# sidward14/gan-lab

Measured on AMD Instinct MI355X. Metric: images/sec (G+D step), StyleGAN 1024^2 bs32/GPU, higher is better.
Workload: dtype f32; 1 GPU; StyleGAN res_samples=1024 FFHQ-shaped synthetic, bs=32/GPU fp32, nonsaturating + R1(lambda=10) + drift, stabilised phase, 1 D-iter + 1 G-iter; global_batch=32, per_gpu_batch=32, parallelism=single

## Files before the change

### gan_lab_amd/_lib.py

```python
import ctypes
import os
import subprocess

import torch

_HERE = os.path.dirname(os.path.abspath(__file__))
CSRC = os.path.join(_HERE, 'csrc')
SO_PATH = os.path.join(CSRC, os.path.basename(os.environ.get('GANLAB_HIP_LIB', '') or 'libganlab_hip.so'))

_c_int, _c_ll, _c_f, _c_p, _c_sz, _c_u64 = (ctypes.c_int, ctypes.c_longlong, ctypes.c_float, ctypes.c_void_p,
                                             ctypes.c_size_t, ctypes.c_uint64)

ACT_NONE, ACT_LRELU = 0, 1
PACK_FWD, PACK_DGRAD = 0, 1


class ConvGeom(ctypes.Structure):
    _fields_ = [('N', _c_int), ('Cin', _c_int), ('Hin', _c_int), ('Win', _c_int),
                ('Cout', _c_int), ('ks', _c_int), ('pad', _c_int), ('up', _c_int), ('pool', _c_int)]


_GP = ctypes.POINTER(ConvGeom)


class PackDesc(ctypes.Structure):
    _fields_ = [('src', _c_p), ('dst', _c_p), ('kind', _c_int), ('Cout', _c_int), ('Cin', _c_int), ('ks', _c_int),
                ('mode', _c_int), ('up', _c_int), ('scale', _c_f), ('reserved', _c_int), ('total', _c_ll),
                ('block0', _c_ll)]

class SnJob(ctypes.Structure):
    _fields_ = [('w', _c_p), ('w_sn', _c_p), ('g_sn', _c_p), ('gw', _c_p), ('u', _c_p), ('v', _c_p), ('sigma', _c_p),
                ('tpart', _c_p), ('s', _c_p), ('dpart', _c_p), ('R', _c_int), ('K', _c_int), ('blk_t0', _c_ll),
                ('blk_s0', _c_ll), ('blk_e0', _c_ll)]


SN_ROW_CHUNK, SN_COL_TILE, SN_ELEM_BLOCK = 16, 1024, 2048


class OrthoJob(ctypes.Structure):
    _fields_ = [('w', _c_p), ('gw', _c_p), ('s', _c_p), ('q', _c_p), ('part', _c_p), ('penalty', _c_p), ('R', _c_int),
                ('K', _c_int), ('form', _c_int), ('n_part', _c_int), ('blk_g0', _c_ll), ('blk_a0', _c_ll)]


class EwmaJob(ctypes.Structure):
    _fields_ = [('dst', _c_p), ('src', _c_p), ('count', _c_ll)]


ORTHO_TILE, ORTHO_QROWS, ORTHO_ROW, ORTHO_COL = 64, 4, 0, 1


class HierJob(ctypes.Structure):
    _fields_ = [('w', _c_p), ('gw', _c_p), ('gw_own', _c_p), ('C', _c_int), ('z_off', _c_int), ('z_len', _c_int),
                ('col', _c_int), ('scale', _c_f), ('one', _c_f), ('blk_f0', _c_ll), ('blk_w0', _c_ll)]


SIGNATURES = {
    'ganlab_abi_version': (_c_int, []),
    'ganlab_last_launch': (_c_int, [ctypes.c_char_p, _c_int, ctypes.POINTER(ctypes.c_uint)]),
    'ganlab_launch_count': (ctypes.c_ulonglong, []),
    'ganlab_launch_history': (_c_int, [_c_int, ctypes.c_char_p, _c_int, ctypes.POINTER(ctypes.c_uint)]),
    'ganlab_conv_geom_size': (_c_int, []),
    'ganlab_conv_out_hw': (_c_int, [_GP, ctypes.POINTER(_c_int), ctypes.POINTER(_c_int)]),
    'ganlab_conv_pack_f32': (_c_ll, [_c_p, _c_p, _c_int, _c_int, _c_int, _c_int, _c_f, _c_p]),
    'ganlab_conv_fwd_f32': (_c_int, [_c_p, _c_p, _c_p, _c_p, _GP, _c_f, _c_int, _c_f, _c_p]),
    'ganlab_conv_dgrad_f32': (_c_int, [_c_p, _c_p, _c_p, _GP, _c_p]),
    'ganlab_conv_splitk_plan': (_c_int, [_GP, _c_int]),
    'ganlab_conv_fwd_splitk_f32': (_c_int, [_c_p, _c_p, _c_p, _c_p, _GP, _c_f, _c_int, _c_f, _c_p, _c_sz, _c_p]),
    'ganlab_conv_dgrad_splitk_f32': (_c_int, [_c_p, _c_p, _c_p, _GP, _c_p, _c_sz, _c_p]),
    'ganlab_conv_dgrad_mask_supported': (_c_int, [_GP]),
    'ganlab_conv_dgrad_mask_f32': (_c_int, [_c_p, _c_p, _c_p, _c_p, _GP, _c_f, _c_p]),
    'ganlab_conv_act_bwd_fused_supported': (_c_int, [_GP]),
    'ganlab_conv_dgrad_act_f32': (_c_int, [_c_p, _c_p, _c_p, _c_p, _GP, _c_f, _c_p]),
    'ganlab_conv_fwd_mask_f32': (_c_int, [_c_p, _c_p, _c_p, _c_p, _GP, _c_f, _c_p]),
    'ganlab_conv_wgrad_act_f32': (_c_int, [_c_p, _c_p, _c_p, _c_p, _c_p, _GP, _c_f, _c_f, _c_f, _c_p, _c_sz, _c_p]),
    'ganlab_conv_wgrad_workspace': (_c_sz, [_GP]),
    'ganlab_conv_wgrad_f32': (_c_int, [_c_p, _c_p, _c_p, _GP, _c_f, _c_p, _c_sz, _c_p]),
    'ganlab_conv_s2_supported': (_c_int, [_GP]),
    'ganlab_conv_s2_pack_f32': (_c_ll, [_c_p, _c_p, _c_int, _c_int, _c_int, _c_int, _c_f, _c_p]),
    'ganlab_conv_s2_fwd_f32': (_c_int, [_c_p, _c_p, _c_p, _c_p, _GP, _c_f, _c_int, _c_f, _c_p]),
    'ganlab_conv_s2_dgrad_f32': (_c_int, [_c_p, _c_p, _c_p, _GP, _c_p]),
    'ganlab_conv_s2_wgrad_workspace': (_c_sz, [_GP]),
    'ganlab_conv_s2_wgrad_f32': (_c_int, [_c_p, _c_p, _c_p, _GP, _c_f, _c_p, _c_sz, _c_p]),
    'ganlab_conv_bf16_supported': (_c_int, [_GP]),
    'ganlab_conv_pack_bf16': (_c_ll, [_c_p, _c_p, _c_int, _c_int, _c_int, _c_f, _c_p]),
    'ganlab_conv_fwd_bf16': (_c_int, [_c_p, _c_p, _c_p, _c_p, _GP, _c_f, _c_int, _c_f, _c_p]),
    'ganlab_conv_dgrad_bf16': (_c_int, [_c_p, _c_p, _c_p, _GP, _c_p]),
    'ganlab_conv_bf16_splitk_plan': (_c_int, [_GP, _c_int]),
    'ganlab_conv_fwd_bf16_splitk': (_c_int, [_c_p, _c_p, _c_p, _c_p, _GP, _c_f, _c_int, _c_f, _c_p, _c_sz, _c_p]),
    'ganlab_conv_dgrad_bf16_splitk': (_c_int, [_c_p, _c_p, _c_p, _GP, _c_p, _c_sz, _c_p]),
    'ganlab_conv_wgrad_bf16_workspace': (_c_sz, [_GP]),
    'ganlab_conv_wgrad_bf16': (_c_int, [_c_p, _c_p, _c_p, _GP, _c_f, _c_p, _c_sz, _c_p]),
    'ganlab_conv_x3_supported': (_c_int, [_GP, _c_int]),
    'ganlab_conv_x3_pack': (_c_ll, [_c_p, _c_p, _c_int, _c_int, _c_int, _c_f, _c_p]),
    'ganlab_conv_fwd_x3': (_c_int, [_c_p, _c_p, _c_p, _c_p, _GP, _c_f, _c_int, _c_f, _c_p]),
    'ganlab_conv_dgrad_x3': (_c_int, [_c_p, _c_p, _c_p, _GP, _c_p]),
    'ganlab_conv_dgrad_mask_x3': (_c_int, [_c_p, _c_p, _c_p, _c_p, _GP, _c_f, _c_p]),
    'ganlab_conv_fwd_aff_x3': (_c_int, [_c_p, _c_p, _c_p, _c_p, _c_p, _c_p, _GP, _c_f, _c_int, _c_f, _c_p]),
    'ganlab_conv_fwd_aff_tail_x3_chunks': (_c_int, [_GP]),
    'ganlab_conv_s2_x3_supported': (_c_int, [_GP, _c_int]),
    'ganlab_conv_s2_x3_pack': (_c_ll, [_c_p, _c_p, _c_int, _c_int, _c_int, _c_f, _c_p]),
    'ganlab_conv_s2_fwd_x3': (_c_int, [_c_p, _c_p, _c_p, _c_p, _GP, _c_f, _c_int, _c_f, _c_p]),
    'ganlab_conv_s2_fwd_aff_x3': (_c_int, [_c_p, _c_p, _c_p, _c_p, _c_p, _c_p, _GP, _c_f, _c_int, _c_f, _c_p]),
    'ganlab_conv_s2_dgrad_x3': (_c_int, [_c_p, _c_p, _c_p, _GP, _c_p]),
    'ganlab_conv_s2_down_x3_supported': (_c_int, [_GP, _c_int]),
    'ganlab_conv_s2_down_x3_pack': (_c_ll, [_c_p, _c_p, _c_int, _c_int, _c_int, _c_f, _c_p]),
    'ganlab_conv_s2_down_fwd_x3': (_c_int, [_c_p, _c_p, _c_p, _c_p, _GP, _c_f, _c_int, _c_f, _c_p]),
    'ganlab_conv_s2_down_dgrad_x3': (_c_int, [_c_p, _c_p, _c_p, _GP, _c_p]),
    'ganlab_conv_wgrad_x3_supported': (_c_int, [_GP]),
    'ganlab_conv_wgrad_x3_workspace': (_c_sz, [_GP]),
    'ganlab_conv_wgrad_x3': (_c_int, [_c_p, _c_p, _c_p, _c_p, _c_p, _GP, _c_f, _c_p, _c_sz, _c_p]),
    'ganlab_conv_s2_wgrad_x3_supported': (_c_int, [_GP]),
    'ganlab_conv_s2_wgrad_x3_workspace': (_c_sz, [_GP]),
    'ganlab_conv_s2_wgrad_x3': (_c_int, [_c_p, _c_p, _c_p, _c_p, _c_p, _GP, _c_f, _c_p, _c_sz, _c_p]),
    'ganlab_conv_fwd_aff_tail_x3': (_c_int, [_c_p, _c_p, _c_p, _c_p, _c_p, _c_p, _c_p, _c_p, _c_p, _c_p, _GP, _c_f, _c_int, _c_f,
                                             _c_f, _c_p, _c_sz, _c_p]),
    'ganlab_mask_bits_supported': (_c_int, [_c_int, _c_int]),
    'ganlab_blur3x3_bits_f32': (_c_int, [_c_p, _c_p, _c_p, _c_ll, _c_int, _c_int, _c_p]),
    'ganlab_blur_act_bwd_bits_f32': (_c_int, [_c_p, _c_p, _c_p, _c_p, _c_int, _c_int, _c_int, _c_int, _c_f, _c_f,
                                              _c_p, _c_sz, _c_p]),
    'ganlab_act_bwd_blur_bits_f32': (_c_int, [_c_p, _c_p, _c_p, _c_p, _c_p, _c_p, _c_int, _c_int, _c_int, _c_int,
                                              _c_f, _c_f, _c_p, _c_sz, _c_p]),
    'ganlab_conv_fwd_blur_supported': (_c_int, [_GP, _c_p, _c_p]),
    'ganlab_conv_fwd_blur_bits_f32': (_c_int, [_c_p, _c_p, _c_p, _c_p, _c_p, _GP, _c_f, _c_f, _c_p]),
    'ganlab_conv_s2_blur_supported': (_c_int, [_GP]),
    'ganlab_conv_s2_blur_workspace': (_c_sz, [_GP]),
    'ganlab_conv_s2_fwd_blur_tail_f32': (_c_int, [_c_p, _c_p, _c_p, _c_p, _c_p, _c_p, _c_p, _c_p, _c_p, _c_p, _GP, _c_f, _c_int,
                                                  _c_f, _c_f, _c_p, _c_sz, _c_p]),
    'ganlab_conv_s2_dgrad_blur_act_bits_f32': (_c_int, [_c_p, _c_p, _c_p, _c_p, _c_p, _GP, _c_f, _c_f, _c_p, _c_sz, _c_p]),
    'ganlab_conv_dgrad_rgb_sums_supported': (_c_int, [_GP, _c_int]),
    'ganlab_conv_dgrad_rgb_sums_workspace': (_c_sz, [_GP]),
    'ganlab_conv_dgrad_rgb_sums_f32': (_c_int, [_c_p, _c_p, _c_p, _c_p, _c_p, _c_p, _GP, _c_int, _c_f, _c_f, _c_f, _c_int, _c_int,
                                                _c_p, _c_sz, _c_p]),
    'ganlab_conv_fwd_bits_f32': (_c_int, [_c_p, _c_p, _c_p, _c_p, _c_p, _GP, _c_f, _c_int, _c_f, _c_p]),
    'ganlab_conv_dgrad_act_bits_f32': (_c_int, [_c_p, _c_p, _c_p, _c_p, _GP, _c_f, _c_p]),
    'ganlab_conv_fwd_mask_bits_f32': (_c_int, [_c_p, _c_p, _c_p, _c_p, _GP, _c_f, _c_p]),
    'ganlab_conv_wgrad_act_bits_f32': (_c_int, [_c_p, _c_p, _c_p, _c_p, _c_p, _GP, _c_f, _c_f, _c_f, _c_p, _c_sz, _c_p]),
    'ganlab_pack_desc_size': (_c_int, []),
    'ganlab_pack_many': (_c_int, [_c_p, _c_int, _c_ll, _c_p]),
    'ganlab_in_affine_f32': (_c_int, [_c_p, _c_p, _c_p, _c_p, _c_p, _c_int, _c_int, _c_p]),
    'ganlab_conv_aff_supported': (_c_int, [_GP]),
    'ganlab_conv_fwd_aff_f32': (_c_int, [_c_p, _c_p, _c_p, _c_p, _c_p, _c_p, _GP, _c_f, _c_int, _c_f, _c_p]),
    'ganlab_conv_fwd_aff_tail_chunks': (_c_int, [_GP]),
    'ganlab_conv_fwd_aff_tail_f32': (_c_int, [_c_p, _c_p, _c_p, _c_p, _c_p, _c_p, _c_p, _c_p, _c_p, _c_p, _GP, _c_f, _c_int, _c_f,
                                              _c_f, _c_p, _c_sz, _c_p]),
    'ganlab_conv_wgrad_aff_f32': (_c_int, [_c_p, _c_p, _c_p, _c_p, _c_p, _GP, _c_f, _c_p, _c_sz, _c_p]),
    'ganlab_conv_s2_aff_supported': (_c_int, [_GP]),
    'ganlab_conv_s2_fwd_aff_f32': (_c_int, [_c_p, _c_p, _c_p, _c_p, _c_p, _c_p, _GP, _c_f, _c_int, _c_f, _c_p]),
    'ganlab_conv_s2_wgrad_aff_f32': (_c_int, [_c_p, _c_p, _c_p, _c_p, _c_p, _GP, _c_f, _c_p, _c_sz, _c_p]),
    'ganlab_mod_conv_supported': (_c_int, [_GP]),
    'ganlab_mod_conv_stat_chunks': (_c_int, [_GP]),
    'ganlab_mod_conv_fwd_f32': (_c_int, [_c_p, _c_p, _c_p, _c_p, _c_p, _c_p, _c_p, _c_p, _c_p, _c_p, _GP, _c_f, _c_int,
                                         _c_f, _c_f, _c_p, _c_sz, _c_p]),
    'ganlab_mod_torgb_prep_f32': (_c_int, [_c_p, _c_p, _c_p, _c_p, _c_p, _c_p, _c_int, _c_int, _c_int, _c_f, _c_f, _c_p]),
    'ganlab_mod_torgb_wgrad_f32': (_c_int, [_c_p, _c_p, _c_p, _c_p, _c_p, _c_int, _c_int, _c_int, _c_f, _c_f, _c_p]),
    'ganlab_mod_torgb_fwd_f32': (_c_int, [_c_p, _c_p, _c_p, _c_p, _c_int, _c_int, _c_int, _c_ll, _c_p]),
    'ganlab_mod_torgb_cross_workspace': (_c_sz, [_c_int]),
    'ganlab_mod_torgb_cross_f32': (_c_int, [_c_p, _c_p, _c_p, _c_int, _c_int, _c_int, _c_ll, _c_p, _c_sz, _c_p]),
    'ganlab_blur3x3_f32': (_c_int, [_c_p, _c_p, _c_ll, _c_int, _c_int, _c_p]),
    'ganlab_up2_f32': (_c_int, [_c_p, _c_p, _c_ll, _c_int, _c_int, _c_f, _c_p]),
    'ganlab_pool2_f32': (_c_int, [_c_p, _c_p, _c_ll, _c_int, _c_int, _c_f, _c_p]),
    'ganlab_resample2d_f32': (_c_int, [_c_p, _c_p, _c_p, _c_p, _c_p, _c_p, _c_ll, _c_int, _c_int, _c_int, _c_int, _c_int,
                                       _c_int, _c_p]),
    'ganlab_bias_act_f32': (_c_int, [_c_p, _c_p, _c_p, _c_p, _c_p, _c_int, _c_int, _c_ll, _c_f, _c_int, _c_f, _c_p]),
    'ganlab_act_bwd_f32': (_c_int, [_c_p, _c_p, _c_p, _c_ll, _c_f, _c_p]),
    'ganlab_act_bwd_bias_f32': (_c_int, [_c_p, _c_p, _c_p, _c_p, _c_int, _c_int, _c_ll, _c_f, _c_f, _c_p, _c_sz, _c_p]),
    'ganlab_channel_sum_f32': (_c_int, [_c_p, _c_p, _c_p, _c_int, _c_int, _c_ll, _c_f, _c_p, _c_sz, _c_p]),
    'ganlab_channel_sum_workspace': (_c_sz, [_c_int, _c_int, _c_ll]),
    'ganlab_instnorm_stats_f32': (_c_int, [_c_p, _c_p, _c_p, _c_ll, _c_ll, _c_f, _c_p]),
    'ganlab_row_stats_workspace': (_c_sz, [_c_ll, _c_ll]),
    'ganlab_row_stats_f32': (_c_int, [_c_p, _c_p, _c_p, _c_ll, _c_ll, _c_f, _c_p, _c_sz, _c_p]),
    'ganlab_instnorm_style_fwd_f32': (_c_int, [_c_p, _c_p, _c_p, _c_p, _c_p, _c_int, _c_int, _c_ll, _c_p]),
    'ganlab_instnorm_style_bwd_reduce_f32': (_c_int, [_c_p, _c_p, _c_p, _c_p, _c_p, _c_p, _c_ll, _c_ll, _c_p]),
    'ganlab_instnorm_style_bwd_apply_f32': (_c_int, [_c_p, _c_p, _c_p, _c_p, _c_p, _c_p, _c_p, _c_p, _c_int, _c_int,
                                                     _c_ll, _c_p]),
    'ganlab_pixelnorm_fwd_f32': (_c_int, [_c_p, _c_p, _c_int, _c_int, _c_ll, _c_f, _c_p]),
    'ganlab_pixelnorm_bwd_f32': (_c_int, [_c_p, _c_p, _c_p, _c_int, _c_int, _c_ll, _c_f, _c_p]),
    'ganlab_blur_fused_supported': (_c_int, [_c_int, _c_int]),
    'ganlab_blur_fused_workspace': (_c_sz, [_c_int, _c_int, _c_int, _c_int]),
    'ganlab_blur_bias_act_f32': (_c_int, [_c_p, _c_p, _c_p, _c_p, _c_p, _c_int, _c_int, _c_int, _c_int, _c_f,
                                          _c_int, _c_f, _c_p]),
    'ganlab_blur_act_bwd_f32': (_c_int, [_c_p, _c_p, _c_p, _c_p, _c_int, _c_int, _c_int, _c_int, _c_f, _c_f,
                                         _c_p, _c_sz, _c_p]),
    'ganlab_act_bwd_blur_f32': (_c_int, [_c_p, _c_p, _c_p, _c_p, _c_p, _c_p, _c_int, _c_int, _c_int, _c_int,
                                         _c_f, _c_f, _c_p, _c_sz, _c_p]),
    'ganlab_act_stats_workspace': (_c_sz, [_c_int, _c_int, _c_ll]),
    'ganlab_bias_act_stats_f32': (_c_int, [_c_p, _c_p, _c_p, _c_p, _c_p, _c_p, _c_p, _c_int, _c_int, _c_ll, _c_f, _c_int,
                                           _c_f, _c_f, _c_p, _c_sz, _c_p]),
    'ganlab_blur_bias_act_stats_f32': (_c_int, [_c_p, _c_p, _c_p, _c_p, _c_p, _c_p, _c_p, _c_int, _c_int, _c_int, _c_int,
                                                _c_f, _c_int, _c_f, _c_f, _c_p, _c_sz, _c_p]),
    'ganlab_instnorm_bwd_act_workspace': (_c_sz, [_c_int, _c_int, _c_ll]),
    'ganlab_instnorm_style_bwd_act_f32': (_c_int, [_c_p] * 11 + [_c_int, _c_int, _c_ll, _c_int, _c_f, _c_f, _c_p, _c_sz,
                                                                 _c_p]),
    'ganlab_instnorm_bwd_rgb_supported': (_c_int, [_c_int, _c_int, _c_int, _c_ll]),
    'ganlab_instnorm_bwd_reduce_rgb_workspace': (_c_sz, [_c_int, _c_int, _c_ll]),
    'ganlab_instnorm_style_bwd_reduce_rgb_f32': (_c_int, [_c_p, _c_p, _c_int] + [_c_p] * 5 + [_c_int, _c_int, _c_ll, _c_p,
                                                                                            _c_sz, _c_p]),
    'ganlab_instnorm_style_bwd_act_rgb_f32': (_c_int, [_c_p, _c_p, _c_int] + [_c_p] * 10 + [_c_int, _c_int, _c_ll, _c_int,
                                                                                         _c_f, _c_f, _c_p, _c_sz, _c_p]),
    'ganlab_instnorm_style_bwd_act_blur_f32': (_c_int, [_c_p] * 11 + [_c_int, _c_int, _c_int, _c_int, _c_int, _c_f, _c_f,
                                                                      _c_p, _c_sz, _c_p]),
    'ganlab_u8_box_decode_f32': (_c_int, [_c_p, _c_p, _c_int, _c_int, _c_int, _c_int, _c_int, _c_p, _c_p, _c_p, _c_p]),
    'ganlab_chan_affine_f32': (_c_int, [_c_p, _c_p, _c_p, _c_p, _c_int, _c_int, _c_ll, _c_p]),
    'ganlab_mul_f32': (_c_int, [_c_p, _c_p, _c_p, _c_ll, _c_p]),
    'ganlab_ln_affine_fwd_f32': (_c_int, [_c_p, _c_p, _c_p, _c_p, _c_p, _c_p, _c_int, _c_ll, _c_int, _c_f, _c_p]),
    'ganlab_colscale_f32': (_c_int, [_c_p, _c_p, _c_p, _c_int, _c_ll, _c_p]),
    'ganlab_coldot_f32': (_c_int, [_c_p, _c_p, _c_p, _c_p, _c_p, _c_p, _c_int, _c_ll, _c_p]),
    'ganlab_ln_rowsums_workspace': (_c_sz, [_c_int, _c_ll]),
    'ganlab_ln_rowsums_f32': (_c_int, [_c_p, _c_p, _c_p, _c_p, _c_p, _c_p, _c_p, _c_p, _c_int, _c_ll, _c_p, _c_sz, _c_p, _c_p,
                                       _c_f, _c_p]),
    'ganlab_ln_project_f32': (_c_int, [_c_p, _c_p, _c_p, _c_p, _c_p, _c_p, _c_p, _c_p, _c_int, _c_ll, _c_p]),
    'ganlab_ln_bwd_cols_f32': (_c_int, [_c_p, _c_p, _c_p, _c_p, _c_p, _c_p, _c_p, _c_p, _c_p, _c_int, _c_ll, _c_p]),
    'ganlab_ln_bwdbwd_apply_f32': (_c_int, [_c_p, _c_p, _c_p, _c_p, _c_p, _c_p, _c_p, _c_p, _c_int, _c_ll, _c_p]),
    'ganlab_bn_stats_f32': (_c_int, [_c_p, _c_p, _c_int, _c_int, _c_ll, _c_p, _c_sz, _c_p]),
    'ganlab_bn_finalize_f32': (_c_int, [_c_p, _c_p, _c_p, _c_p, _c_p, _c_p, _c_int, _c_f, _c_f, _c_f, _c_p]),
    'ganlab_bn_apply_f32': (_c_int, [_c_p, _c_p, _c_p, _c_p, _c_p, _c_int, _c_int, _c_ll, _c_int, _c_f, _c_p]),
    'ganlab_bn_bwd_sums_f32': (_c_int, [_c_p, _c_p, _c_p, _c_p, _c_p, _c_int, _c_int, _c_ll, _c_p, _c_sz, _c_p, _c_p, _c_f,
                                        _c_p]),
    'ganlab_bn_bwd_apply_f32': (_c_int, [_c_p, _c_p, _c_p, _c_p, _c_p, _c_p, _c_p, _c_int, _c_int, _c_ll, _c_p]),
    'ganlab_tanh_fwd_f32': (_c_int, [_c_p, _c_p, _c_ll, _c_p]),
    'ganlab_tanh_bwd_f32': (_c_int, [_c_p, _c_p, _c_p, _c_ll, _c_p]),
    'ganlab_mbstd_fwd_f32': (_c_int, [_c_p, _c_p, _c_int, _c_int, _c_ll, _c_f, _c_p]),
    'ganlab_mbstd_bwd_f32': (_c_int, [_c_p, _c_p, _c_p, _c_int, _c_int, _c_ll, _c_f, _c_p]),
    'ganlab_mbstd_bwdbwd_f32': (_c_int, [_c_p, _c_p, _c_p, _c_p, _c_p, _c_int, _c_int, _c_ll, _c_f, _c_p]),
    'ganlab_axpby_f32': (_c_int, [_c_p, _c_p, _c_p, _c_ll, _c_f, _c_f, _c_p]),
    'ganlab_scale_dev_f32': (_c_int, [_c_p, _c_p, _c_p, _c_ll, _c_f, _c_p]),
    'ganlab_lerp_rows_f32': (_c_int, [_c_p, _c_p, _c_p, _c_p, _c_ll, _c_ll, _c_p]),
    'ganlab_sum_f32': (_c_int, [_c_p, _c_p, _c_ll, _c_f, _c_int, _c_p, _c_sz, _c_p]),
    'ganlab_sum_workspace': (_c_sz, [_c_ll]),
    'ganlab_bce_logits_fwd_f32': (_c_int, [_c_p, _c_p, _c_int, _c_f, _c_p]),
    'ganlab_bce_logits_bwd_f32': (_c_int, [_c_p, _c_p, _c_p, _c_int, _c_f, _c_p]),
    'ganlab_hinge_fwd_f32': (_c_int, [_c_p, _c_p, _c_int, _c_f, _c_f, _c_p]),
    'ganlab_hinge_bwd_f32': (_c_int, [_c_p, _c_p, _c_p, _c_int, _c_f, _c_f, _c_p]),
    'ganlab_chnorm_penalty_fwd_f32': (_c_int, [_c_p, _c_p, _c_int, _c_int, _c_ll, _c_f, _c_f, _c_p, _c_sz, _c_p]),
    'ganlab_chnorm_penalty_bwd_f32': (_c_int, [_c_p, _c_p, _c_p, _c_int, _c_int, _c_ll, _c_f, _c_f, _c_p]),
    'ganlab_adam_f32': (_c_int, [_c_p, _c_p, _c_p, _c_p, _c_ll, _c_f, _c_f, _c_f, _c_f, _c_f, _c_f, _c_f, _c_p]),
    'ganlab_ewma_f32': (_c_int, [_c_p, _c_p, _c_ll, _c_f, _c_p]),
    'ganlab_randn_f32': (_c_int, [_c_p, _c_ll, _c_u64, _c_u64, _c_p]),
    'ganlab_randn_dev_f32': (_c_int, [_c_p, _c_ll, _c_u64, _c_p, _c_u64, _c_p]),
    'ganlab_diffaug_params_f32': (_c_int, [_c_p, _c_int, _c_int, _c_int, _c_u64, _c_u64, _c_p]),
    'ganlab_diffaug_params_dev_f32': (_c_int, [_c_p, _c_int, _c_int, _c_int, _c_u64, _c_p, _c_u64, _c_p]),
    'ganlab_diffaug_fwd_workspace': (_c_sz, [_c_int, _c_int, _c_int, _c_int]),
    'ganlab_diffaug_bwd_workspace': (_c_sz, [_c_int, _c_int, _c_int, _c_int]),
    'ganlab_diffaug_fwd_f32': (_c_int, [_c_p, _c_p, _c_p, _c_int, _c_int, _c_int, _c_int, _c_p, _c_sz, _c_p]),
    'ganlab_diffaug_bwd_f32': (_c_int, [_c_p, _c_p, _c_p, _c_int, _c_int, _c_int, _c_int, _c_p, _c_sz, _c_p]),
    'ganlab_ada_params_f32': (_c_int, [_c_p, _c_int, _c_int, _c_int, _c_p, _c_int, _c_u64, _c_u64, _c_p]),
    'ganlab_ada_params_dev_f32': (_c_int, [_c_p, _c_int, _c_int, _c_int, _c_p, _c_int, _c_u64, _c_p, _c_u64, _c_p]),
    'ganlab_ada_fwd_f32': (_c_int, [_c_p, _c_p, _c_p, _c_int, _c_int, _c_int, _c_p]),
    'ganlab_ada_bwd_f32': (_c_int, [_c_p, _c_p, _c_p, _c_int, _c_int, _c_int, _c_p]),
    'ganlab_ada_update_f32': (_c_int, [_c_p, _c_p, _c_int, _c_int, _c_f, _c_f, _c_p]),
    'ganlab_swd_down_f32': (_c_int, [_c_p, _c_p, _c_ll, _c_int, _c_int, _c_p]),
    'ganlab_swd_band_f32': (_c_int, [_c_p, _c_p, _c_p, _c_ll, _c_int, _c_int, _c_p]),
# ... 149 lines not shown
```

### gan_lab_amd/csrc/common.h

```cpp
#pragma once
#include <hip/hip_runtime.h>
#include <stdint.h>

#include "../../include/ganlab_hip.h"

typedef float f32x4 __attribute__((ext_vector_type(4)));

static thread_local int gl_launch_status = GANLAB_OK;
extern thread_local const void* gl_last_kernel_fn;
extern thread_local unsigned gl_last_grid;
#define GL_LAUNCH_RING 16
extern thread_local const void* gl_ring_fn[GL_LAUNCH_RING];
extern thread_local unsigned gl_ring_grid[GL_LAUNCH_RING];
extern thread_local unsigned long long gl_launch_count;
#define GL_LAUNCH(k, grid, ...)                                                  \
  do {                                                                           \
    (void)hipGetLastError();                                                     \
    const dim3 gl_grid_ = (grid);                                                \
    gl_last_kernel_fn = reinterpret_cast<const void*>(k);                        \
    gl_last_grid = gl_grid_.x * gl_grid_.y * gl_grid_.z;                         \
    gl_ring_fn[gl_launch_count % GL_LAUNCH_RING] = gl_last_kernel_fn;            \
    gl_ring_grid[gl_launch_count % GL_LAUNCH_RING] = gl_last_grid;               \
    ++gl_launch_count;                                                           \
    hipLaunchKernelGGL(k, gl_grid_, __VA_ARGS__);                                \
    if (hipGetLastError() != hipSuccess) gl_launch_status = GANLAB_ELAUNCH;      \
  } while (0)
static inline int gl_take_status() {
  const int s = gl_launch_status;
  gl_launch_status = GANLAB_OK;
  return s;
}
#define GL_CHECK_LAUNCH() gl_take_status()

#include <cstdlib>
#define GL_ENV_ONCE(name) ([]() -> const char* { static const char* const v = getenv(name); return v; }())

static inline hipStream_t gl_stream(void* s) { return reinterpret_cast<hipStream_t>(s); }

__device__ __forceinline__ int gl_xcd_remap(int b, int n) {
  const int q = n >> 3, r = n & 7, xcd = b & 7, i = b >> 3;
  const int base = (xcd < r) ? xcd * (q + 1) : r * (q + 1) + (xcd - r) * q;
  return base + i;
}

__device__ __forceinline__ float gl_wave_sum(float v) {
#pragma unroll
  for (int o = 32; o > 0; o >>= 1) v += __shfl_xor(v, o, 64);
  return v;
}

__device__ __forceinline__ float gl_block_sum_256(float v, float* red) {
  v = gl_wave_sum(v);
  __syncthreads();
  if ((threadIdx.x & 63) == 0) red[threadIdx.x >> 6] = v;
  __syncthreads();
  return red[0] + red[1] + red[2] + red[3];
}

__device__ __forceinline__ double gl_block_sum_256d(double v, double* red) {
#pragma unroll
  for (int o = 32; o > 0; o >>= 1) v += __shfl_xor(v, o, 64);
  __syncthreads();
  if ((threadIdx.x & 63) == 0) red[threadIdx.x >> 6] = v;
  __syncthreads();
  return (red[0] + red[1]) + (red[2] + red[3]);
}

#ifndef GL_ACC_DUMP
#define GL_ACC_DUMP 1
#endif
#ifndef GL_ACC_DUMP_TERMS_V
#define GL_ACC_DUMP_TERMS_V 144
#endif
constexpr int GL_ACC_DUMP_TERMS = GL_ACC_DUMP_TERMS_V;

__device__ __forceinline__ void philox4x32_10(uint32_t c[4], uint32_t k0, uint32_t k1) {
#pragma unroll
  for (int r = 0; r < 10; ++r) {
    const uint64_t p0 = (uint64_t)0xD2511F53u * c[0], p1 = (uint64_t)0xCD9E8D57u * c[2];
    const uint32_t n0 = (uint32_t)(p1 >> 32) ^ c[1] ^ k0, n1 = (uint32_t)p1;
    const uint32_t n2 = (uint32_t)(p0 >> 32) ^ c[3] ^ k1, n3 = (uint32_t)p0;
    c[0] = n0; c[1] = n1; c[2] = n2; c[3] = n3;
    k0 += 0x9E3779B9u;
    k1 += 0xBB67AE85u;
  }
}

__device__ __forceinline__ float gl_lrelu(float v, float slope) { return v > 0.f ? v : v * slope; }

__device__ __forceinline__ float4 gl_few_dot(const float4 (&xv)[4], const float* __restrict__ wp, int Cin, int Cout_p, int co,
                                             float start) {
  float4 a = float4{start, start, start, start};
#pragma unroll
  for (int ci = 0; ci < 4; ++ci) {
    const float w = ci < Cin ? wp[(long long)ci * Cout_p + co] : 0.f;
    a.x += w * xv[ci].x; a.y += w * xv[ci].y; a.z += w * xv[ci].z; a.w += w * xv[ci].w;
  }
  return a;
}

struct gl_bf16x3 { __bf16 h, m, l; };
__device__ __forceinline__ gl_bf16x3 gl_split3(float v) {
  const __bf16 h = (__bf16)v;
  const float r1 = v - (float)h;
  const __bf16 m = (__bf16)r1;
  return gl_bf16x3{h, m, (__bf16)(r1 - (float)m)};
}

__device__ __forceinline__ void gl_x3_pack_position(const float* __restrict__ w9, bool flip, float scale, __bf16* __restrict__ out,
                                                    int CI, int ci, int co) {
  const int steps = CI / 32 * 9;
  const int ct = co >> 6, col = co & 63, c = ci >> 5, half = (ci >> 4) & 1, g = (ci >> 3) & 1, j = ci & 7;
#pragma unroll
  for (int t = 0; t < 9; ++t) {
    const int s = t < 8 ? (half ? 5 : 0) + (t >> 1) : 4;
    const int hi = t < 8 ? (t & 1) : half;
    const int kg = hi * 2 + g;
    float v = w9[flip ? 8 - t : t] * scale;
    asm volatile("" : "+v"(v));
    const gl_bf16x3 p = gl_split3(v);
    __bf16* base = out + (((long long)ct * steps + c * 9 + s) * (3 * 4 * 64)) * 8;
    base[((0 * 4 + kg) * 64 + col) * 8 + j] = p.h;
    base[((1 * 4 + kg) * 64 + col) * 8 + j] = p.m;
    base[((2 * 4 + kg) * 64 + col) * 8 + j] = p.l;
  }
}

__device__ __forceinline__ void gl_x3_up_pack_position(const float* __restrict__ w9, int up, float scale, __bf16* __restrict__ out,
                                                       int CI, int CO, int ci, int co) {
  const int nsteps = CI / 8;
  const bool c32 = (CO & 63) != 0;
  const int ct = c32 ? co >> 5 : co >> 6, j = ci & 7;
#pragma unroll
  for (int py = 0; py < 2; ++py)
#pragma unroll
    for (int px = 0; px < 2; ++px)
#pragma unroll
      for (int ty = 0; ty < 2; ++ty)
#pragma unroll
        for (int tx = 0; tx < 2; ++tx) {
          float v = 0.f;
#pragma unroll
          for (int ky = 0; ky < 3; ++ky)
#pragma unroll
            for (int kx = 0; kx < 3; ++kx) {
              const int ry = up ? ky : 2 - ky, rx = up ? kx : 2 - kx;
              const bool iny = py == 0 ? (ty == 0 ? ry == 0 : ry >= 1) : (ty == 0 ? ry <= 1 : ry == 2);
              const bool inx = px == 0 ? (tx == 0 ? rx == 0 : rx >= 1) : (tx == 0 ? rx <= 1 : rx == 2);
              if (iny && inx) v += w9[ky * 3 + kx];
            }
          v = v * (up ? scale : 0.25f * scale);
          asm volatile("" : "+v"(v));
          const gl_bf16x3 p = gl_split3(v);
          __bf16* base = out + (((c32 ? (long long)ct : (long long)ct * 2 + py) * nsteps + (ci >> 3)) * (3 * 4 * 128)) * 8;
          const int col = c32 ? py * 32 + (co & 31) : co & 63;
          const int kgq = ty * 2 + tx;
          base[((0 * 4 + kgq) * 128 + px * 64 + col) * 8 + j] = p.h;
          base[((1 * 4 + kgq) * 128 + px * 64 + col) * 8 + j] = p.m;
          base[((2 * 4 + kgq) * 128 + px * 64 + col) * 8 + j] = p.l;
        }
}

__device__ __forceinline__ float gl_comb_s2(int up, int a, int k) {
  if (up) {
    const int lo = (a == 0) ? 2 : (a == 1 ? 1 : 0), hi = (a == 0) ? 2 : (a == 1 ? 2 : (a == 2 ? 1 : 0));
    return (k >= lo && k <= hi) ? 1.f : 0.f;
  }
  const int lo = (a <= 1) ? 0 : (a == 2 ? 1 : 2), hi = (a == 0) ? 0 : (a == 1 ? 1 : 2);
  return (k >= lo && k <= hi) ? 0.5f : 0.f;
}
__device__ __forceinline__ void gl_x3_down_pack_position(const float* __restrict__ w9, int up, float scale, __bf16* __restrict__ out,
                                                         int CI, int ci, int co) {
  const int nsteps = CI / 8 * 4;
  const int ct = co >> 7, col = co & 127, q = ci >> 3, j = ci & 7;
  float k9[9];
#pragma unroll
  for (int t = 0; t < 9; ++t) k9[t] = w9[t];
#pragma unroll
  for (int a = 0; a < 4; ++a)
#pragma unroll
    for (int b = 0; b < 4; ++b) {
      float v = 0.f;
#pragma unroll
      for (int ky = 0; ky < 3; ++ky)
#pragma unroll
        for (int kx = 0; kx < 3; ++kx) v += gl_comb_s2(up, a, ky) * gl_comb_s2(up, b, kx) * k9[ky * 3 + kx];
      v = v * scale;
      asm volatile("" : "+v"(v));
      const gl_bf16x3 p = gl_split3(v);
      __bf16* base = out + (((long long)ct * nsteps + q * 4 + a) * (3 * 4 * 128)) * 8;
      base[((0 * 4 + b) * 128 + col) * 8 + j] = p.h;
      base[((1 * 4 + b) * 128 + col) * 8 + j] = p.m;
      base[((2 * 4 + b) * 128 + col) * 8 + j] = p.l;
    }
}

extern "C" int gl_tail_stats_finish(const double* spart, float* mean, float* rstd, long long planes, int chunks, double inv_hw, float eps,
                         hipStream_t st);

bool gl_wgrad_roll_supported(int N, int Cin, int Cout, int H, int W, int ks, int pad, int up, const void* x,
                             const void* gy);
int gl_wgrad_roll_slots(int N, int Cin, int Cout, int H, int W);
int gl_wgrad_roll_launch(const float* x, const float* gy, float* part, int N, int Cin, int Cout, int H, int W,
                         hipStream_t st, const float* aff_s = nullptr, const float* aff_t = nullptr);
bool gl_wgrad_s2_roll_supported(int N, int Cl, int Ch, int Hl, int Wl, const void* low, const void* high);
int gl_wgrad_s2_roll_slots(int N, int Cl, int Ch, int Hl, int Wl);
int gl_wgrad_s2_roll_launch(const float* low, const float* high, float* part, int N, int Cl, int Ch, int Hl, int Wl,
                            hipStream_t st, const float* aff_s = nullptr, const float* aff_t = nullptr);

bool gl_s2_roll_supported(int is_T, int N, int Cin, int Cout, int Hl, int Wl, const void* x, const void* y);
int gl_s2_roll_launch(int is_T, const float* x, const float* wp, const float* bias, float* y, int N, int Cin, int Cout,
                      int Hl, int Wl, int Cin_p, int Cout_p, float bias_scale, int act, float slope, hipStream_t st,
                      const float* aff_s = nullptr, const float* aff_t = nullptr);

bool gl_roll_blur_supported(int N, int Cin, int Cout, int H, int W, const void* x, const void* y);
int gl_roll_blur_launch(const float* x, const float* wp, const float* bias, float* y, void* bits, int N, int Cin, int Cout,
                        int H, int W, int Cin_p, int Cout_p, float bias_scale, float slope, hipStream_t st, int blur, int act);
```

### gan_lab_amd/csrc/conv_x3.hip

```cpp
#include "x3_common.h"

#include <type_traits>

#ifndef X3_EXP
#define X3_EXP 0
#endif

namespace {

constexpr int X3_NT = 64;
constexpr int X3_PL = 336;
constexpr int X3_HALF = 6 * X3_PL;
constexpr int X3_WSTEP = 3 * 4 * X3_NT;
constexpr int X3_AOFF = 0, X3_WOFF = 3 * X3_HALF;
constexpr int X3_WSTAGE = 2 * X3_WSTEP;
constexpr int X3_LDS = 3 * X3_HALF + 2 * X3_WSTAGE;

__host__ __device__ constexpr int x3_tap_lo(int s) { return s < 4 ? 2 * s : s == 4 ? 8 : 2 * (s - 5); }
__host__ __device__ constexpr int x3_tap_hi(int s) { return s < 4 ? 2 * s + 1 : s == 4 ? 8 : 2 * (s - 5) + 1; }
__host__ __device__ constexpr int x3_half_lo(int s) { return s <= 4 ? 0 : 1; }
__host__ __device__ constexpr int x3_half_hi(int s) { return s < 4 ? 0 : 1; }

__global__ void x3_pack_kernel(const float* __restrict__ w, __bf16* __restrict__ out, int Cout, int Cin, int mode, float scale) {
  const bool dg = mode == GANLAB_PACK_DGRAD;
  const int CO = dg ? Cin : Cout, CI = dg ? Cout : Cin;
  const long long e = blockIdx.x * (long long)blockDim.x + threadIdx.x;
  if (e >= (long long)CO * CI) return;
  const int col = (int)(e & 63);
  const long long t = e >> 6;
  const int ci = (int)(t % CI), ct = (int)(t / CI);
  const int co = ct * 64 + col;
  const float* w9 = dg ? w + ((long long)ci * Cin + co) * 9 : w + ((long long)co * Cin + ci) * 9;
  gl_x3_pack_position(w9, dg, scale, out, CI, ci, co);
}

struct X3Args {
  const float* x;
  const u32x4* wp;
  const float* bias;
  float* y;
  int N, CI, CO, H, W;
  int tiles_x, tiles_y, tiles_co, ntiles;
  float bias_scale, slope;
  int act;
  const float* mask;
  float mslope;
  const float* aff_s;
  const float* aff_t;
  const float* noise;
  const float* noise_w;
  double* spart;
};

constexpr int X3_PLAIN = 0, X3_MASK = 1, X3_AFF = 2, X3_AFF_TAIL = 3;

#define X3_ACC8(a) "+v"(a[0][0]), "+v"(a[0][1]), "+v"(a[1][0]), "+v"(a[1][1]), "+v"(a[2][0]), "+v"(a[2][1]), "+v"(a[3][0]), "+v"(a[3][1])

__host__ __device__ constexpr int x3_toff(int tap) { return (tap / 3) * 18 + tap % 3; }

struct X3Tile { int n, oy0, ox0, co_t; };

template <int FORM>
__global__ __launch_bounds__(512) void conv_x3_fwd_kernel(X3Args p) {
  constexpr bool MASK = FORM == X3_MASK, AFF = FORM == X3_AFF || FORM == X3_AFF_TAIL, TAIL = FORM == X3_AFF_TAIL;
  constexpr int NLOADS = AFF ? 6 : 4;
  __shared__ __attribute__((aligned(16))) u32x4 lds[X3_LDS];

  const int tid = threadIdx.x, lane = tid & 63;
  const int wv = __builtin_amdgcn_readfirstlane(tid >> 6);
  const int wm = wv >> 1, wn = wv & 1;
  const int l16 = lane & 15, kg = lane >> 4, lane16 = lane * 16;
  const int plane = p.H * p.W;
  const int nstages = p.CI / 64 * 9, ndc = p.CI / 64;
  const int G = gridDim.x;

  auto decode = [&](int t) {
    X3Tile c;
    c.co_t = t % p.tiles_co; t /= p.tiles_co;
    c.ox0 = (t % p.tiles_x) * 16; t /= p.tiles_x;
    c.oy0 = (t % p.tiles_y) * 16;
    c.n = t / p.tiles_y;
    return c;
  };

  const bool a_item = tid < 432;
  int a_pack;
  {
    const int e = a_item ? tid : 0;
    const int cq = e & 1;
    int t = e >> 1;
    const int cg = t % 6; t /= 6;
    const int r = t % 18, g = t / 18;
    const int unit48 = ((g * 3) * X3_PL + r * 18 + 4 * cg) * 16 + cq * 8;
    a_pack = unit48 | ((cg == 0 ? 3 : 0) << 16) | ((cg == 5 ? 1 : 4) << 18) | (r << 21) | (cg << 26) | ((g * 2 + cq) << 29);
  }
  const int cstride = plane * 4;
  f32x4 ar[4];
  f32x4 a_sv, a_tv;
  auto a_load = [&](const X3Tile& c, int half) {
    const u32x4 rs = x3_rsrc(p.x + (long long)c.n * p.CI * plane, (unsigned)((long long)p.CI * plane * 4));
    int pk = a_pack;
    asm volatile("" : "+v"(pk));
    const int ry = ((pk >> 21) & 31) - 1, rx = ((pk >> 26) & 7) * 4 - 4, a_ch = ((pk >> 29) & 3) * 4;
    const bool ok = a_item && (unsigned)(c.oy0 + ry) < (unsigned)p.H && (unsigned)(c.ox0 + rx) < (unsigned)p.W;
    const int off = ok ? (a_ch * plane + (c.oy0 + ry) * p.W + c.ox0 + rx) * 4 : (int)0x80000000;
    const int soff = half * 16 * plane * 4;
    if (X3_EXP & 4) return;
#pragma unroll
    for (int j = 0; j < 4; ++j) x3_ld(ar[j], rs, off + j * cstride, soff);
    if constexpr (AFF) {
      const unsigned tab = (unsigned)((long long)p.N * p.CI * 4);
      const u32x4 rss = x3_rsrc(p.aff_s, tab), rst = x3_rsrc(p.aff_t, tab);
      const int o = ok ? a_ch * 4 : (int)0x80000000;
      const int so = (c.n * p.CI + half * 16) * 4;
      x3_ld(a_sv, rss, o, so);
      x3_ld(a_tv, rst, o, so);
    }
  };
  auto a_wait = [&](auto younger) {
    if constexpr (AFF) x3_ld_wait<decltype(younger)::value>(ar, a_sv, a_tv); else x3_ld_wait<decltype(younger)::value>(ar);
  };
  auto a_store_px = [&](int slot, int i) {
    if (!a_item || (X3_EXP & 1)) return;
    int pk = a_pack;
    asm volatile("" : "+v"(pk));
    const int a_i0 = (pk >> 16) & 3, a_i1 = (pk >> 18) & 7;
    unsigned char* dst = reinterpret_cast<unsigned char*>(lds + X3_AOFF + slot * X3_HALF) + ((pk & 0x7fff) - 48);
    if (i < a_i0 || i >= a_i1) return;
    bf16x4 h, m, l;
#pragma unroll
    for (int j = 0; j < 4; ++j) {
      float v = i == 0 ? ar[j].x : i == 1 ? ar[j].y : i == 2 ? ar[j].z : ar[j].w;
      if constexpr (AFF) v = fmaf(v, j == 0 ? a_sv.x : j == 1 ? a_sv.y : j == 2 ? a_sv.z : a_sv.w,
                                  j == 0 ? a_tv.x : j == 1 ? a_tv.y : j == 2 ? a_tv.z : a_tv.w);
      x3_split_lane(v, j, h, m, l);
    }
    *reinterpret_cast<u32x2*>(dst + i * 16) = __builtin_bit_cast(u32x2, h);
    *reinterpret_cast<u32x2*>(dst + i * 16 + X3_PL * 16) = __builtin_bit_cast(u32x2, m);
    *reinterpret_cast<u32x2*>(dst + i * 16 + 2 * X3_PL * 16) = __builtin_bit_cast(u32x2, l);
  };
  auto a_store = [&](int slot) {
#pragma unroll
    for (int i = 0; i < 4; ++i) {
      a_store_px(slot, i);
      __builtin_amdgcn_sched_barrier(0);
    }
  };

  const __amdgpu_buffer_rsrc_t rs_w = __builtin_amdgcn_make_buffer_rsrc(
      const_cast<u32x4*>(p.wp), 0, (unsigned)((long long)p.tiles_co * nstages * X3_WSTAGE * 16), 0x00020000);
  auto w_dma = [&](const X3Tile& c, int st, int buf) {
    const int soff = (c.co_t * nstages + st) * (X3_WSTAGE * 16) + wv * 3072;
#pragma unroll
    for (int i = 0; i < 3; ++i)
      __builtin_amdgcn_raw_ptr_buffer_load_lds(rs_w, (__attribute__((address_space(3))) void*)(lds + X3_WOFF + buf * X3_WSTAGE + wv * 192 + i * 64),
                                               16, lane16, soff + i * 1024, 0, 0);
  };

  f32x4 accS[4][2], accH[4][2], accT[4][2];
#pragma unroll
  for (int m = 0; m < 4; ++m)
#pragma unroll
    for (int nn = 0; nn < 2; ++nn) {
      accS[m][nn] = f32x4{0.f, 0.f, 0.f, 0.f}; accH[m][nn] = f32x4{0.f, 0.f, 0.f, 0.f}; accT[m][nn] = f32x4{0.f, 0.f, 0.f, 0.f};
    }

  const int laneA = X3_AOFF + (kg & 1) * 3 * X3_PL + (4 * wm) * 18 + l16;
  const int laneB = X3_WOFF + kg * X3_NT + wn * 32 + l16;
  const bool khi = kg >= 2;
  const int khi_i = khi ? 1 : 0;

  bf16x8 aF[2][3], bF[2][2][3];
  auto a_frags = [&](int off, int m) {
#pragma unroll
    for (int pl = 0; pl < 3; ++pl) aF[m & 1][pl] = __builtin_bit_cast(bf16x8, lds[off + pl * X3_PL + m * 18]);
  };
  auto b_frags = [&](int buf, int step1, int nn, int set) {
#pragma unroll
    for (int pl = 0; pl < 3; ++pl)
      bF[set][nn][pl] = __builtin_bit_cast(bf16x8, lds[laneB + buf * X3_WSTAGE + step1 * X3_WSTEP + pl * 4 * X3_NT + nn * 16]);
  };

  int tile = gl_xcd_remap(blockIdx.x, G);
  if (tile >= p.ntiles) return;
  X3Tile cur = decode(tile);

  w_dma(cur, 0, 0);
  a_load(cur, 0); a_wait(std::integral_constant<int, 0>{}); a_store(0);
  a_load(cur, 1); a_wait(std::integral_constant<int, 0>{}); a_store(1);
  x3_barrier<0>();
  if (nstages > 1) w_dma(cur, 1, 1);
  int offA;
  {
    offA = laneA + (khi ? x3_toff(x3_tap_hi(0)) : x3_toff(x3_tap_lo(0)));
    a_frags(offA, 0);
    b_frags(0, 0, 0, 0);
    b_frags(0, 0, 1, 0);
  }

  int st = 0;
  int gst = 0;
  int r0 = 0;
  for (;;) {
    const int ntile = tile + G;
    const bool nvalid = ntile < p.ntiles;
    const X3Tile nxt = decode(nvalid ? ntile : tile);
    for (int dc = 0; dc < ndc; ++dc) {
      const int sl0 = r0, sl1 = r0 == 2 ? 0 : r0 + 1, sl2 = sl1 == 2 ? 0 : sl1 + 1;
      const bool lastdc = dc + 1 == ndc;
      const bool more = !lastdc || nvalid;
#pragma unroll
// ... 264 lines not shown
```

### gan_lab_amd/csrc/pack.hip

```cpp
#include "common.h"

namespace {

constexpr int round_up_c(int v, int m) { return (v + m - 1) / m * m; }

__global__ __launch_bounds__(256) void pack_many_kernel(const ganlab_pack_desc* __restrict__ descs, int n_desc) {
  int lo = 0, hi = n_desc - 1;
  const long long b = blockIdx.x;
  while (lo < hi) {
    const int mid = (lo + hi + 1) >> 1;
    if (descs[mid].block0 <= b) lo = mid; else hi = mid - 1;
  }
  const ganlab_pack_desc d = descs[lo];
  const long long e = (b - d.block0) * 256 + threadIdx.x;
  const float* w = d.src;
  if (d.kind == GANLAB_PACKKIND_PLAIN) {
    const int KK = d.ks * d.ks, dgrad = d.mode == GANLAB_PACK_DGRAD;
    const int rows = dgrad ? d.Cout : d.Cin, cols = dgrad ? d.Cin : d.Cout;
    const int rows_p = round_up_c(rows, d.ks == 1 ? 32 : 16), cols_p = round_up_c(cols, 64);
    const long long plane = (long long)rows_p * cols_p;
    if (e >= plane) return;
    const int col = (int)(e % cols_p), row = (int)(e / cols_p);
    const bool in = row < rows && col < cols;
    const int co = dgrad ? row : col, ci = dgrad ? col : row;
    const float* ws = w + ((long long)co * d.Cin + ci) * KK;
    float* out = reinterpret_cast<float*>(d.dst) + e;
    for (int tap = 0; tap < KK; ++tap)
      out[tap * plane] = in ? d.scale * ws[dgrad ? (KK - 1 - tap) : tap] : 0.f;
  } else if (d.kind == GANLAB_PACKKIND_S2) {
    const int transpose = d.mode;
    const int rows = transpose ? d.Cout : d.Cin, cols = transpose ? d.Cin : d.Cout;
    const int rows_p = round_up_c(rows, 16), cols_p = round_up_c(cols, 64);
    const long long plane = (long long)rows_p * cols_p;
    if (e >= plane) return;
    const int col = (int)(e % cols_p), row = (int)(e / cols_p);
    const bool in = row < rows && col < cols;
    const int co = transpose ? row : col, ci = transpose ? col : row;
    float k9[9];
    const float* ws = w + ((long long)co * d.Cin + ci) * 9;
#pragma unroll
    for (int t = 0; t < 9; ++t) k9[t] = in ? ws[t] : 0.f;
    float* out = reinterpret_cast<float*>(d.dst) + e;
#pragma unroll
    for (int tap = 0; tap < 16; ++tap) {
      const int a = tap >> 2, bb = tap & 3;
      float v = 0.f;
#pragma unroll
      for (int ky = 0; ky < 3; ++ky)
#pragma unroll
        for (int kx = 0; kx < 3; ++kx) v += gl_comb_s2(d.up, a, ky) * gl_comb_s2(d.up, bb, kx) * k9[ky * 3 + kx];
      out[tap * plane] = v * d.scale;
    }
  } else if (d.kind == GANLAB_PACKKIND_X3 && d.ks == 4) {
    const int up = d.up;
    const int CO = up ? d.Cout : d.Cin, CI = up ? d.Cin : d.Cout;
    if (e >= (long long)CO * CI) return;
    int ci, co;
    if ((CO & 63) == 0) {
      const int col = (int)(e & 63);
      const long long t = e >> 6;
      ci = (int)(t % CI);
      co = (int)(t / CI) * 64 + col;
    } else {
      co = (int)(e % CO);
      ci = (int)(e / CO);
    }
    const float* w9 = up ? w + ((long long)co * d.Cin + ci) * 9 : w + ((long long)ci * d.Cin + co) * 9;
    gl_x3_up_pack_position(w9, up, d.scale, reinterpret_cast<__bf16*>(d.dst), CI, CO, ci, co);
  } else if (d.kind == GANLAB_PACKKIND_X3 && d.ks == 5) {
    const int up = d.up;
    const int CO = up ? d.Cin : d.Cout, CI = up ? d.Cout : d.Cin;
    if (e >= (long long)CO * CI) return;
    const int col = (int)(e & 127);
    const long long t = e >> 7;
    const int ci = (int)(t % CI), ct = (int)(t / CI);
    const int co = ct * 128 + col;
    const float* w9 = up ? w + ((long long)ci * d.Cin + co) * 9 : w + ((long long)co * d.Cin + ci) * 9;
    gl_x3_down_pack_position(w9, up, d.scale, reinterpret_cast<__bf16*>(d.dst), CI, ci, co);
  } else if (d.kind == GANLAB_PACKKIND_X3) {
    const bool dg = d.mode == GANLAB_PACK_DGRAD;
    const int CO = dg ? d.Cin : d.Cout, CI = dg ? d.Cout : d.Cin;
    if (e >= (long long)CO * CI) return;
    const int col = (int)(e & 63);
    const long long t = e >> 6;
    const int ci = (int)(t % CI), ct = (int)(t / CI);
    const int co = ct * 64 + col;
    const float* w9 = dg ? w + ((long long)ci * d.Cin + co) * 9 : w + ((long long)co * d.Cin + ci) * 9;
    gl_x3_pack_position(w9, dg, d.scale, reinterpret_cast<__bf16*>(d.dst), CI, ci, co);
  } else {
    const int dg = d.mode == GANLAB_PACK_DGRAD;
    const int CO = dg ? d.Cin : d.Cout;
    if (e >= d.total / 9) return;
    const int j = (int)(e & 7);
    long long t = e >> 3;
    const int co = (int)(t % CO);
    t /= CO;
    const int kg = (int)(t & 3);
    const int chunk = (int)(t >> 2);
    const int ci = chunk * 32 + kg * 8 + j;
    const float* ws = dg ? w + ((long long)ci * d.Cin + co) * 9 : w + ((long long)co * d.Cin + ci) * 9;
    __bf16* out = reinterpret_cast<__bf16*>(d.dst);
#pragma unroll
    for (int tap = 0; tap < 9; ++tap)
      out[((((long long)chunk * 9 + tap) * 4 + kg) * CO + co) * 8 + j] = (__bf16)(ws[dg ? 8 - tap : tap] * d.scale);
  }
}

}

extern "C" {

int ganlab_pack_desc_size(void) { return (int)sizeof(ganlab_pack_desc); }

int ganlab_pack_many(const ganlab_pack_desc* descs_device, int n_desc, long long total_blocks, void* stream) {
  if (!descs_device || n_desc <= 0 || total_blocks <= 0 || total_blocks > 0x7fffffffLL) return GANLAB_EINVAL;
  GL_LAUNCH(pack_many_kernel, dim3((unsigned)total_blocks), dim3(256), 0, gl_stream(stream), descs_device, n_desc);
  return GL_CHECK_LAUNCH();
}

}
```

### gan_lab_amd/csrc/x3_common.h

```cpp
#pragma once
#include "common.h"

namespace {

typedef __bf16 bf16x8 __attribute__((ext_vector_type(8)));
typedef __bf16 bf16x4 __attribute__((ext_vector_type(4)));
typedef unsigned int u32x4 __attribute__((ext_vector_type(4)));
typedef unsigned int u32x2 __attribute__((ext_vector_type(2)));

__device__ __forceinline__ u32x4 x3_rsrc(const void* base, unsigned bytes) {
  const unsigned long long b = reinterpret_cast<unsigned long long>(base);
  return u32x4{(unsigned)__builtin_amdgcn_readfirstlane((int)(unsigned)b), (unsigned)__builtin_amdgcn_readfirstlane((int)(unsigned)(b >> 32)) & 0xffffu,
               (unsigned)__builtin_amdgcn_readfirstlane((int)bytes), 0x00020000u};
}
__device__ __forceinline__ void x3_ld(f32x4& d, const u32x4& rs, int voff, int soff) {
  asm volatile("buffer_load_dwordx4 %0, %1, %2, %3 offen" : "=v"(d) : "v"(voff), "s"(rs), "s"(soff));
}
__device__ __forceinline__ void x3_ld(f32x4& d, const u32x4& rs, int voff) {
  asm volatile("buffer_load_dwordx4 %0, %1, %2, 0 offen" : "=v"(d) : "v"(voff), "s"(rs));
}
template <int YOUNGER>
__device__ __forceinline__ void x3_ld_wait(f32x4 (&a)[4]) {
  asm volatile("s_waitcnt vmcnt(%4)" : "+v"(a[0]), "+v"(a[1]), "+v"(a[2]), "+v"(a[3]) : "n"(YOUNGER));
}
template <int YOUNGER>
__device__ __forceinline__ void x3_ld_wait(f32x4 (&a)[4], f32x4& s_, f32x4& t_) {
  asm volatile("s_waitcnt vmcnt(%6)" : "+v"(a[0]), "+v"(a[1]), "+v"(a[2]), "+v"(a[3]), "+v"(s_), "+v"(t_) : "n"(YOUNGER));
}
template <int YOUNGER>
__device__ __forceinline__ void x3_ld_wait(f32x4& a, f32x4& b) {
  asm volatile("s_waitcnt vmcnt(%2)" : "+v"(a), "+v"(b) : "n"(YOUNGER));
}

template <int YOUNGER>
__device__ __forceinline__ void x3_barrier() {
  if constexpr (YOUNGER == 0) asm volatile("s_waitcnt vmcnt(0) lgkmcnt(0)\n\ts_barrier" ::: "memory");
  else if constexpr (YOUNGER == 4) asm volatile("s_waitcnt vmcnt(4) lgkmcnt(0)\n\ts_barrier" ::: "memory");
  else asm volatile("s_waitcnt vmcnt(6) lgkmcnt(0)\n\ts_barrier" ::: "memory");
  static_assert(YOUNGER == 0 || YOUNGER == 4 || YOUNGER == 6, "an activation staging issues four loads (six with the affine)");
}

#define X3_MFMA(acc, a, b) asm volatile("v_mfma_f32_16x16x32_bf16 %0, %1, %2, %0" : "+v"(acc) : "v"(a), "v"(b))
#define X3_DRAIN(...) asm volatile("s_nop 15\n\ts_nop 15" : __VA_ARGS__)
#define X3_SETTLE(...) asm volatile("s_nop 7\n\ts_nop 7" : __VA_ARGS__)

__device__ __forceinline__ void x3_split_lane(float v, int j, bf16x4& h, bf16x4& m, bf16x4& l) {
  h[j] = (__bf16)v;
  const float r1 = v - (float)h[j];
  m[j] = (__bf16)r1;
  l[j] = (__bf16)(r1 - (float)m[j]);
}
__device__ __forceinline__ void x3_split4(const f32x4& v, u32x2& h, u32x2& m, u32x2& l) {
  bf16x4 hh, mm, ll;
#pragma unroll
  for (int j = 0; j < 4; ++j) x3_split_lane(v[j], j, hh, mm, ll);
  h = __builtin_bit_cast(u32x2, hh); m = __builtin_bit_cast(u32x2, mm); l = __builtin_bit_cast(u32x2, ll);
}

}
```

### gan_lab_amd/ops.py

```python
import ctypes
import os

import numpy as np

import torch
from torch.autograd import Function
from torch.autograd.function import once_differentiable

from . import _lib
from ._lib import ACT_LRELU, ACT_NONE, PACK_DGRAD, PACK_FWD, ConvGeom, check


def _p(t):
    return ctypes.c_void_p(t.data_ptr()) if t is not None else None


_RAW_STREAM = getattr(torch._C, '_cuda_getCurrentRawStream', None)
_GET_DEVICE = getattr(torch._C, '_cuda_getDevice', None)


def _st():
    if _RAW_STREAM is None or _GET_DEVICE is None:
        return ctypes.c_void_p(torch.cuda.current_stream().cuda_stream)
    return ctypes.c_void_p(_RAW_STREAM(_GET_DEVICE()))
# ... 31 lines not shown
        raise TypeError(f'gan_lab_amd.ops: {what} draws on the GPU (got device {device!r}); the HIP path has no CPU fallback')


def _new(shape, like):
    return torch.empty(shape, dtype=torch.float32, device=like.device)


_COMPUTE = ['f32']


def set_compute_dtype(name):
    if name not in ('f32', 'bf16'):
        raise ValueError("compute dtype must be 'f32' or 'bf16'")
    _COMPUTE[0] = name


def get_compute_dtype():
    return _COMPUTE[0]


class compute_dtype(object):

    def __init__(self, name):
        self.name = name

    def __enter__(self):
        self._prev = _COMPUTE[0]
        set_compute_dtype(self.name)

    def __exit__(self, *exc):
        _COMPUTE[0] = self._prev
        return False


class Geom:
    __slots__ = ('N', 'Cin', 'Hin', 'Win', 'Cout', 'ks', 'pad', 'up', 'pool', 'Ho', 'Wo', 's2', '_c', 'bf', 'bf_fused')

    _CACHE = {}

    def __new__(cls, N, Cin, Hin, Win, Cout, ks, pad, up=0, pool=0):
        key = (int(N), int(Cin), int(Hin), int(Win), int(Cout), int(ks), int(pad), int(bool(up)), int(bool(pool)),
               _COMPUTE[0])
        g = cls._CACHE.get(key)
        if g is None:
            g = object.__new__(cls)
            g._c = None
            g._build(*key[:9])
            if len(cls._CACHE) > 4096:
                cls._CACHE.clear()
            cls._CACHE[key] = g
        return g

    def __init__(self, N, Cin, Hin, Win, Cout, ks, pad, up=0, pool=0):
        pass

    def _build(self, N, Cin, Hin, Win, Cout, ks, pad, up, pool):
        if ks not in (1, 3):
            raise ValueError('conv kernels support ks in {1, 3}; a 4x4 valid conv runs as a linear')
        self.N, self.Cin, self.Hin, self.Win, self.Cout, self.ks, self.pad, self.up, self.pool = \
            int(N), int(Cin), int(Hin), int(Win), int(Cout), int(ks), int(pad), int(bool(up)), int(bool(pool))
        hv, wv = (2 * Hin, 2 * Win) if up else (Hin, Win)
        self.Ho, self.Wo = hv + 2 * pad - ks + 1, wv + 2 * pad - ks + 1
        if self.pool:
            self.Ho, self.Wo = self.Ho // 2, self.Wo // 2
        cg = ConvGeom(self.N, self.Cin, self.Hin, self.Win, self.Cout, self.ks, self.pad, self.up, self.pool)
        self.bf = self.bf_fused = None
        if _COMPUTE[0] == 'bf16':
            v = ConvGeom(self.N, self.Cin, hv, wv, self.Cout, self.ks, self.pad, 0, 0)
            if _lib.lib().ganlab_conv_bf16_supported(ctypes.byref(v)):
                self.bf = v
                if (self.up or self.pool) and _lib.lib().ganlab_conv_bf16_supported(ctypes.byref(cg)):
                    self.bf_fused = cg
                elif self.pool:
                    self.bf = None
        self.s2 = bool(self.bf is None and (self.up or self.pool) and
                       _lib.lib().ganlab_conv_s2_supported(ctypes.byref(cg)))
        if self.pool and not self.s2 and self.bf_fused is None:
            raise ValueError('pool=1 geometry is not supported by the stride-2 kernels; compose conv + pool')
        self._c = cg

    def ref(self):
        return ctypes.byref(self._c)

    @property
    def in_shape(self):
        return (self.N, self.Cin, self.Hin, self.Win)

    @property
    def out_shape(self):
        return (self.N, self.Cout, self.Ho, self.Wo)


def pool_fusable(N, Cin, Hin, Win, Cout, ks, pad):
    if ks != 3 or pad != 1:
        return False
    if _COMPUTE[0] == 'bf16':
        v = ConvGeom(int(N), int(Cin), int(Hin), int(Win), int(Cout), 3, 1, 0, 1)
        if _lib.lib().ganlab_conv_bf16_supported(ctypes.byref(v)):
            return True
    c = ConvGeom(int(N), int(Cin), int(Hin), int(Win), int(Cout), 3, 1, 0, 1)
    return bool(_lib.lib().ganlab_conv_s2_supported(ctypes.byref(c)))


class _PackEntry(object):
    __slots__ = ('w', 'out', 'serial', 'ptr', 'desc')


_PACK_CACHE = {}
_PACK_SERIAL = [0]
_PACK_GEN = [0]
_PACK_RANGES = {}
_PACK_TABLES = {}
_KIND_PLAIN, _KIND_S2, _KIND_BF16, _KIND_X3 = 0, 1, 2, 3


def bump_weight_epoch(ranges=None):
    _PACK_SERIAL[0] += 1
    if ranges is None:
        if _PACK_CACHE or _PACK_TABLES:
            _PACK_GEN[0] += 1
        _PACK_CACHE.clear()
        _PACK_TABLES.clear()
        _PACK_RANGES.clear()
        return
    for r in ranges:
        _PACK_RANGES[(int(r[0]), int(r[1]))] = _PACK_SERIAL[0]


def pack_generation():
    return _PACK_GEN[0]


_ALL_ADDRESSES = (0, 1 << 62)


def mark_packs_stale():
    if _PACK_RANGES:
        bump_weight_epoch(list(_PACK_RANGES.keys()))
    elif _PACK_CACHE:
        bump_weight_epoch([_ALL_ADDRESSES])


def _pack_one(e):
    L = _lib.lib()
    kind, cout, cin, ks, mode, up, scale, total = e.desc
    if kind == _KIND_S2:
        rc = L.ganlab_conv_s2_pack_f32(_p(e.w), _p(e.out), cout, cin, up, mode, scale, _st())
    elif kind == _KIND_BF16:
        rc = L.ganlab_conv_pack_bf16(_p(e.w), e.out.data_ptr(), cout, cin, mode, scale, _st())
    elif kind == _KIND_X3 and ks == 4:
        rc = L.ganlab_conv_s2_x3_pack(_p(e.w), e.out.data_ptr(), cout, cin, up, scale, _st())
    elif kind == _KIND_X3 and ks == 5:
        rc = L.ganlab_conv_s2_down_x3_pack(_p(e.w), e.out.data_ptr(), cout, cin, up, scale, _st())
    elif kind == _KIND_X3:
        rc = L.ganlab_conv_x3_pack(_p(e.w), e.out.data_ptr(), cout, cin, mode, scale, _st())
    else:
        rc = L.ganlab_conv_pack_f32(_p(e.w), _p(e.out), cout, cin, ks, mode, scale, _st())
    if rc != total:
        raise _lib.GanlabLibraryError(f're-pack failed ({rc} != {total})')


def _stale_range(e):
    for r, ser in _PACK_RANGES.items():
        if ser > e.serial and r[0] <= e.ptr < r[1]:
            return r
    return None


def _repack_range(r):
    L = _lib.lib()
    ser = _PACK_RANGES[r]
    items = [(k, e) for k, e in _PACK_CACHE.items() if r[0] <= e.ptr < r[1] and e.serial < ser]
    keys = tuple(k for k, _ in items)
    tab = _PACK_TABLES.get(r)
    if (tab is None or tab[0] != keys) and torch.cuda.is_current_stream_capturing():
        for _, e in items:
            _pack_one(e)
            e.serial = _PACK_SERIAL[0]
        return
    if tab is None or tab[0] != keys:
        arr = (_lib.PackDesc * len(items))()
        blocks = 0
        for i, (_, e) in enumerate(items):
            kind, cout, cin, ks, mode, up, scale, total = e.desc
            d = arr[i]
            d.src, d.dst = e.w.data_ptr(), e.out.data_ptr()
            d.kind, d.Cout, d.Cin, d.ks, d.mode, d.up, d.scale, d.total, d.block0 = kind, cout, cin, ks, mode, up, scale, \
                total, blocks
            blocks += (total // (16 if kind == _KIND_S2 else (9 if kind == _KIND_BF16 else ((48 if ks >= 4 else 27) if kind == _KIND_X3 else ks * ks))) + 255) // 256
        host = torch.frombuffer(bytearray(bytes(arr)), dtype=torch.uint8)
        if tab is not None:
            _PACK_GEN[0] += 1
        tab = (keys, host.to(items[0][1].w.device), blocks)
        _PACK_TABLES[r] = tab
    check(L.ganlab_pack_many(tab[1].data_ptr(), len(items), tab[2], _st()), 'pack_many')
    now = _PACK_SERIAL[0]
    for _, e in items:
        e.serial = now


def _pack_lookup(key):
    e = _PACK_CACHE.get(key)
    if e is None:
        return None
    r = _stale_range(e)
    if r is not None:
        _repack_range(r)
    return e.out


def _pack_store(key, w, out, desc):
    if len(_PACK_CACHE) > 1024:
        bump_weight_epoch()
    e = _PackEntry()
    e.w, e.out, e.serial, e.ptr, e.desc = w.detach(), out, _PACK_SERIAL[0], w.data_ptr(), desc
    _PACK_CACHE[key] = e
    return out


def _packed(w, mode, scale, s2_up=None):
    key = (w.data_ptr(), w._version, tuple(w.shape), mode, float(scale), s2_up)
    hit = _pack_lookup(key)
    if hit is not None:
        return hit
    cout, cin, ks = w.shape[0], w.shape[1], w.shape[2]
    L = _lib.lib()
    if s2_up is not None:
        tr = 1 if mode == PACK_DGRAD else 0
        n = L.ganlab_conv_s2_pack_f32(None, None, cout, cin, int(s2_up), tr, scale, None)
        if n <= 0:
            raise _lib.GanlabLibraryError(f'conv_s2_pack size query failed ({n}) for weight {tuple(w.shape)}')
        out = _new((n,), w)
        rc = L.ganlab_conv_s2_pack_f32(_p(w), _p(out), cout, cin, int(s2_up), tr, scale, _st())
        if rc != n:
            raise _lib.GanlabLibraryError(f'conv_s2_pack failed ({rc})')
        return _pack_store(key, w, out, (_KIND_S2, cout, cin, 3, tr, int(s2_up), float(scale), int(n)))
    n = L.ganlab_conv_pack_f32(None, None, cout, cin, ks, mode, scale, None)
    if n <= 0:
        raise _lib.GanlabLibraryError(f'conv_pack size query failed ({n}) for weight {tuple(w.shape)}')
    out = _new((n,), w)
    rc = L.ganlab_conv_pack_f32(_p(w), _p(out), cout, cin, ks, mode, scale, _st())
    if rc != n:
        raise _lib.GanlabLibraryError(f'conv_pack failed ({rc})')
    return _pack_store(key, w, out, (_KIND_PLAIN, cout, cin, ks, mode, 0, float(scale), int(n)))


def _packed_bf16(w, mode, scale):
    key = (w.data_ptr(), w._version, tuple(w.shape), mode, float(scale), 'bf16')
    hit = _pack_lookup(key)
    if hit is not None:
        return hit
    cout, cin = w.shape[0], w.shape[1]
    L = _lib.lib()
    n = L.ganlab_conv_pack_bf16(None, None, cout, cin, mode, scale, None)
    if n <= 0:
        raise _lib.GanlabLibraryError(f'conv_pack_bf16 size query failed ({n}) for weight {tuple(w.shape)}')
    out = torch.empty((n,), dtype=torch.bfloat16, device=w.device)
    rc = L.ganlab_conv_pack_bf16(_p(w), out.data_ptr(), cout, cin, mode, scale, _st())
    if rc != n:
        raise _lib.GanlabLibraryError(f'conv_pack_bf16 failed ({rc})')
    return _pack_store(key, w, out, (_KIND_BF16, cout, cin, 3, mode, 0, float(scale), int(n)))


_X3 = [os.environ.get('GANLAB_X3', '1') != '0']
_X3_MIN_TILES = 128


def set_x3(enabled):
    old = _X3[0]
    _X3[0] = bool(enabled)
    return old


def x3_enabled():
    return _X3[0]


def x3_ok(g, dgrad=False):
    if not _X3[0] or g.bf is not None or g.s2 or g.up or g.pool or g.ks != 3 or g.pad != 1:
        return False
    co = g.Cin if dgrad else g.Cout
    if g.N * (g.Hin // 16) * (g.Win // 16) * (co // 64) < _X3_MIN_TILES:
        return False
    return bool(_lib.lib().ganlab_conv_x3_supported(g.ref(), 1 if dgrad else 0))


def x3_s2_ok(g, dgrad=False):
    if not _X3[0] or not g.s2:
        return False
    if (g.pool if dgrad else g.up) != 1:
        return False
    co = g.Cin if dgrad else g.Cout
    hl, wl = (g.Hin // 2, g.Win // 2) if dgrad else (g.Hin, g.Win)
    if g.N * (hl // 8) * (wl // 16) * (co // 32) < _X3_MIN_TILES:
        return False
    return bool(_lib.lib().ganlab_conv_s2_x3_supported(g.ref(), 1 if dgrad else 0))


def x3_wgrad_ok(g):
    if not _X3[0] or g.bf is not None or g.s2 or g.up or g.pool or g.ks != 3 or g.pad != 1 or g.Cin < 64 or g.Cout < 64:
        return False
    return bool(_lib.lib().ganlab_conv_wgrad_x3_supported(g.ref()))


def _wgrad_x3(gy, x, s_, t_, gw, g, scale):
    L = _lib.lib()
    ws = torch.empty((L.ganlab_conv_wgrad_x3_workspace(g.ref()) + 3) // 4, dtype=torch.float32, device=x.device)
    check(L.ganlab_conv_wgrad_x3(_p(gy), _p(x), _p(s_), _p(t_), _p(gw), g.ref(), scale, _p(ws), ws.numel() * 4, _st()),
          'conv_wgrad_x3')
    return gw


def x3_s2_wgrad_ok(g):
    if not _X3[0] or g.bf is not None or not g.s2 or g.ks != 3 or g.pad != 1:
        return False
    return bool(_lib.lib().ganlab_conv_s2_wgrad_x3_supported(g.ref()))


def _wgrad_x3_s2(gy, x, s_, t_, gw, g, scale):
    L = _lib.lib()
    ws = torch.empty((L.ganlab_conv_s2_wgrad_x3_workspace(g.ref()) + 3) // 4, dtype=torch.float32, device=x.device)
    check(L.ganlab_conv_s2_wgrad_x3(_p(gy), _p(x), _p(s_), _p(t_), _p(gw), g.ref(), scale, _p(ws), ws.numel() * 4, _st()),
          'conv_s2_wgrad_x3')
    return gw


def x3_s2_down_ok(g, dgrad=False):
    if not _X3[0] or not g.s2:
        return False
    if (g.up if dgrad else g.pool) != 1:
        return False
    co = g.Cin if dgrad else g.Cout
    hl, wl = (g.Hin, g.Win) if dgrad else (g.Hin // 2, g.Win // 2)
    if g.N * (hl // 8) * (wl // 16) * (co // 128) < _X3_MIN_TILES:
        return False
    return bool(_lib.lib().ganlab_conv_s2_down_x3_supported(g.ref(), 1 if dgrad else 0))


def _packed_x3_any(name, tag, w, sel, scale, ks):
    key = (w.data_ptr(), w._version, tuple(w.shape), sel, float(scale), tag)
    hit = _pack_lookup(key)
    if hit is not None:
        return hit
    cout, cin = w.shape[0], w.shape[1]
    pack = getattr(_lib.lib(), 'ganlab_' + name)
    n = pack(None, None, cout, cin, sel, scale, None)
    if n <= 0:
        raise _lib.GanlabLibraryError(f'{name} size query failed ({n}) for weight {tuple(w.shape)}')
    out = torch.empty((n,), dtype=torch.bfloat16, device=w.device)
    rc = pack(_p(w), out.data_ptr(), cout, cin, sel, scale, _st())
    if rc != n:
        raise _lib.GanlabLibraryError(f'{name} failed ({rc})')
    mode, up = (sel, 0) if ks == 3 else (0, sel)
    return _pack_store(key, w, out, (_KIND_X3, cout, cin, ks, mode, up, float(scale), int(n)))


def _packed_x3_s2_down(w, up, scale):
    return _packed_x3_any('conv_s2_down_x3_pack', 'x3s2d', w, int(up), scale, 5)


def _packed_x3_s2(w, up, scale):
    return _packed_x3_any('conv_s2_x3_pack', 'x3s2', w, int(up), scale, 4)


def _packed_x3(w, mode, scale):
    return _packed_x3_any('conv_x3_pack', 'x3', w, mode, scale, 3)


_INPUT_GRAD_ONLY = [False]


class input_grad_only(object):
    def __enter__(self):
        self._prev = _INPUT_GRAD_ONLY[0]
        _INPUT_GRAD_ONLY[0] = True

    def __exit__(self, *exc):
        _INPUT_GRAD_ONLY[0] = self._prev
        return False


def _want_param_grads():
    return not _INPUT_GRAD_ONLY[0]


_NO_GRAD_TOWARDS = [None]


class no_grad_towards(object):
    def __init__(self, leaf):
        self.ptr = leaf.data_ptr() if leaf is not None else None

    def __enter__(self):
        self._prev = _NO_GRAD_TOWARDS[0]
        _NO_GRAD_TOWARDS[0] = self.ptr

    def __exit__(self, *exc):
        _NO_GRAD_TOWARDS[0] = self._prev
        return False


def _wants_input_grad(ctx, x):
    return ctx.needs_input_grad[0] and not (_NO_GRAD_TOWARDS[0] is not None and x.grad_fn is None and
                                            x.data_ptr() == _NO_GRAD_TOWARDS[0])


_DIRECT = [False]
_SINK, _TAKEN = {}, {}


def direct_grads_enabled():
    import os
    return os.environ.get('GANLAB_DIRECT_GRADS') != '0'


class direct_param_grads(object):
    def __init__(self, enabled=True):
        self.enabled = bool(enabled)

    def __enter__(self):
        self._prev = _DIRECT[0]
        _DIRECT[0] = self.enabled
        _SINK.clear()
        _TAKEN.clear()

    def __exit__(self, *exc):
        _DIRECT[0] = self._prev
        _SINK.clear()
        _TAKEN.clear()
        return False


def _sink(name, p):
    if not _DIRECT[0] or p is None or torch.is_grad_enabled():
        return
    base = p._base if p._base is not None else p
    arena = getattr(base, '_ganlab_arena', None)
    if arena is None or not base.is_leaf or base.grad is None or base.numel() != p.numel() or \
            getattr(base, '_ganlab_written', -1) == arena.serial:
        return
    _SINK[name] = base


def _take(name, shape, like):
    if _SINK:
        base = _SINK.pop(name, None)
        if base is not None:
            n = 1
            for v in shape:
                n *= int(v)
            if base.grad.numel() == n and base.grad.device == like.device:
                base._ganlab_written = base._ganlab_arena.serial
                _TAKEN[name] = True
                return base.grad.view(shape)
    return _new(shape, like)


def _sunk(name):
    if _SINK:
        _SINK.pop(name, None)
    return _TAKEN.pop(name, False) if _TAKEN else False


_OBSERVER = [None]


def set_launch_observer(fn):
    prev = _OBSERVER[0]
    _OBSERVER[0] = fn
    return prev


def conv_flops(g):
    if g.s2:
        lo_h, lo_w = (g.Hin, g.Win) if g.up else (g.Ho, g.Wo)
        return 2.0 * 16 * g.Cin * g.Cout * lo_h * lo_w * g.N
    if g.bf is not None:
        return 2.0 * g.ks * g.ks * g.Cin * g.Cout * g.bf.Hin * g.bf.Win * g.N
    return 2.0 * g.ks * g.ks * g.Cin * g.Cout * g.Ho * g.Wo * g.N


def _note(kind, g):
    if _OBSERVER[0] is not None:
        _OBSERVER[0](kind, g)


def k_conv_fwd(x, w, bias, g, scale, bias_scale=1.0, act=ACT_NONE, slope=0.2):
    x, w = _c(x, 'conv input'), _c(w, 'conv weight')
    assert tuple(x.shape) == g.in_shape, (tuple(x.shape), g.in_shape)
    assert tuple(w.shape) == (g.Cout, g.Cin, g.ks, g.ks), (tuple(w.shape), g.Cout, g.Cin, g.ks)
    _note('fwd', g)
    if bias is not None:
        bias = _c(bias, 'bias')
        assert bias.numel() == g.Cout
    y = _new(g.out_shape, x)
    if g.bf is not None:
        geom = g.bf_fused if g.bf_fused is not None else g.bf
        xin = k_up2(x, 1.0) if (g.up and g.bf_fused is None) else x
        wp = _packed_bf16(w, PACK_FWD, scale)
        L = _lib.lib()
        split = L.ganlab_conv_bf16_splitk_plan(ctypes.byref(geom), 0)
        if split >= 2:
            m = 2 if geom.up else 1
            ws = torch.empty((split * geom.N * geom.Cout * geom.Hin * m * geom.Win * m,), dtype=torch.float32, device=x.device)
            check(L.ganlab_conv_fwd_bf16_splitk(_p(xin), wp.data_ptr(), _p(bias), _p(y), ctypes.byref(geom), bias_scale, act,
                                                slope, _p(ws), ws.numel() * 4, _st()), 'conv_fwd_bf16_splitk')
            return y
        check(L.ganlab_conv_fwd_bf16(_p(xin), wp.data_ptr(), _p(bias), _p(y), ctypes.byref(geom), bias_scale,
                                     act, slope, _st()), 'conv_fwd_bf16')
        return y
    if x3_s2_down_ok(g):
        check(_lib.lib().ganlab_conv_s2_down_fwd_x3(_p(x), _packed_x3_s2_down(w, 0, scale).data_ptr(), _p(bias), _p(y), g.ref(),
                                                    bias_scale, act, slope, _st()), 'conv_s2_down_fwd_x3')
        return y
    if x3_s2_ok(g):
        check(_lib.lib().ganlab_conv_s2_fwd_x3(_p(x), _packed_x3_s2(w, 1, scale).data_ptr(), _p(bias), _p(y), g.ref(), bias_scale,
                                               act, slope, _st()), 'conv_s2_fwd_x3')
        return y
    if g.s2:
        wp = _packed(w, PACK_FWD, scale, s2_up=g.up)
        check(_lib.lib().ganlab_conv_s2_fwd_f32(_p(x), _p(wp), _p(bias), _p(y), g.ref(), bias_scale, act, slope,
                                                _st()), 'conv_s2_fwd')
        return y
    if g.ks == 1 and g.Hin == 1 and g.Win == 1 and g.N <= 64 and g.Cin >= 2048 and g.Cin % 128 == 0:
        g2 = Geom(1, g.Cout, g.Cin // 128, 128, g.N, 1, 0)
        obs = set_launch_observer(None)
        try:
            y = k_conv_wgrad(x.view(g2.out_shape), w.view(g2.in_shape), g2, scale).view(g.out_shape)
        finally:
            set_launch_observer(obs)
        if bias is not None or act != ACT_NONE:
            y = k_bias_act(y, bias, None, None, bias_scale, act, slope)
        return y
    L = _lib.lib()
    if x3_ok(g):
        check(L.ganlab_conv_fwd_x3(_p(x), _packed_x3(w, PACK_FWD, scale).data_ptr(), _p(bias), _p(y), g.ref(), bias_scale, act,
                                   slope, _st()), 'conv_fwd_x3')
        return y
    wp = _packed(w, PACK_FWD, scale)
    split = 0 if g.up else L.ganlab_conv_splitk_plan(g.ref(), 0)
    if split >= 2:
        ws = torch.empty((split,) + tuple(y.shape), dtype=torch.float32, device=x.device)
        check(L.ganlab_conv_fwd_splitk_f32(_p(x), _p(wp), _p(bias), _p(y), g.ref(), bias_scale, act, slope, _p(ws),
                                           ws.numel() * 4, _st()), 'conv_fwd_splitk')
        return y
    check(L.ganlab_conv_fwd_f32(_p(x), _p(wp), _p(bias), _p(y), g.ref(), bias_scale, act, slope, _st()), 'conv_fwd')
    return y


def k_conv_dgrad(gy, w, g, scale):
    gy, w = _c(gy, 'conv grad_out'), _c(w, 'conv weight')
    assert tuple(gy.shape) == g.out_shape, (tuple(gy.shape), g.out_shape)
    _note('dgrad', g)
    if g.bf is not None:
        wp = _packed_bf16(w, PACK_DGRAD, scale)
        L = _lib.lib()

        def run(geom, out):
            split = L.ganlab_conv_bf16_splitk_plan(ctypes.byref(geom), 1)
            if split >= 2:
                m = 2 if geom.up else 1
                ws = torch.empty((split * geom.N * geom.Cin * geom.Hin * m * geom.Win * m,), dtype=torch.float32,
                                 device=gy.device)
                check(L.ganlab_conv_dgrad_bf16_splitk(_p(gy), wp.data_ptr(), _p(out), ctypes.byref(geom), _p(ws),
                                                      ws.numel() * 4, _st()), 'conv_dgrad_bf16_splitk')
            else:
                check(L.ganlab_conv_dgrad_bf16(_p(gy), wp.data_ptr(), _p(out), ctypes.byref(geom), _st()), 'conv_dgrad_bf16')
            return out
        if g.bf_fused is not None:
            return run(g.bf_fused, _new(g.in_shape, gy))
        gxv = run(g.bf, _new((g.N, g.Cin, g.bf.Hin, g.bf.Win), gy))
        return k_pool2(gxv, 1.0) if g.up else gxv
    if x3_s2_down_ok(g, True):
        gx = _new(g.in_shape, gy)
        check(_lib.lib().ganlab_conv_s2_down_dgrad_x3(_p(gy), _packed_x3_s2_down(w, 1, scale).data_ptr(), _p(gx), g.ref(), _st()),
              'conv_s2_down_dgrad_x3')
        return gx
    if x3_s2_ok(g, True):
        gx = _new(g.in_shape, gy)
        check(_lib.lib().ganlab_conv_s2_dgrad_x3(_p(gy), _packed_x3_s2(w, 0, scale).data_ptr(), _p(gx), g.ref(), _st()),
              'conv_s2_dgrad_x3')
        return gx
    if g.s2:
        wp = _packed(w, PACK_DGRAD, scale, s2_up=g.up)
        gx = _new(g.in_shape, gy)
        check(_lib.lib().ganlab_conv_s2_dgrad_f32(_p(gy), _p(wp), _p(gx), g.ref(), _st()), 'conv_s2_dgrad')
        return gx
    if x3_ok(g, True):
        gx = _new(g.in_shape, gy)
        check(_lib.lib().ganlab_conv_dgrad_x3(_p(gy), _packed_x3(w, PACK_DGRAD, scale).data_ptr(), _p(gx), g.ref(), _st()),
              'conv_dgrad_x3')
        return gx
    wp = _packed(w, PACK_DGRAD, scale)
    hv, wv = (2 * g.Hin, 2 * g.Win) if g.up else (g.Hin, g.Win)
    gxv = _new((g.N, g.Cin, hv, wv), gy)
    split = 0 if g.up else _lib.lib().ganlab_conv_splitk_plan(g.ref(), 1)
    if split >= 2:
        ws = torch.empty((split,) + tuple(gxv.shape), dtype=torch.float32, device=gy.device)
        check(_lib.lib().ganlab_conv_dgrad_splitk_f32(_p(gy), _p(wp), _p(gxv), g.ref(), _p(ws), ws.numel() * 4, _st()),
              'conv_dgrad_splitk')
        return gxv
    check(_lib.lib().ganlab_conv_dgrad_f32(_p(gy), _p(wp), _p(gxv), g.ref(), _st()), 'conv_dgrad')
    if g.up:
        return k_pool2(gxv, 1.0)
    return gxv


def conv_dgrad_mask_ok(g):
    return g.bf is None and not g.s2 and not g.up and bool(_lib.lib().ganlab_conv_dgrad_mask_supported(g.ref()))


def k_conv_dgrad_mask(gy, w, x, g, scale, slope):
    gy, w, x = _c(gy, 'conv grad_out'), _c(w, 'conv weight'), _c(x, 'conv input')
    assert tuple(gy.shape) == g.out_shape and tuple(x.shape) == g.in_shape
    _note('dgrad', g)
    gx = torch.empty_like(x)
    if x3_ok(g, True):
        check(_lib.lib().ganlab_conv_dgrad_mask_x3(_p(gy), _packed_x3(w, PACK_DGRAD, scale).data_ptr(), _p(x), _p(gx), g.ref(),
                                                   slope, _st()), 'conv_dgrad_mask_x3')
        return gx
    check(_lib.lib().ganlab_conv_dgrad_mask_f32(_p(gy), _p(_packed(w, PACK_DGRAD, scale)), _p(x), _p(gx), g.ref(), slope,
                                                _st()), 'conv_dgrad_mask')
    return gx


def conv_act_bwd_fusable(g):
    return g.bf is None and not g.s2 and bool(_lib.lib().ganlab_conv_act_bwd_fused_supported(g.ref()))


def k_conv_dgrad_act(gy, y, w, g, scale, slope):
    gy, w = _c(gy, 'conv grad_out'), _c(w, 'conv weight')
    assert tuple(gy.shape) == g.out_shape
    _note('dgrad', g)
    gx = _new(g.in_shape, gy)
    if _is_bits(y):
        check(_lib.lib().ganlab_conv_dgrad_act_bits_f32(_p(gy), y.data_ptr(), _p(_packed(w, PACK_DGRAD, scale)), _p(gx),
                                                        g.ref(), slope, _st()), 'conv_dgrad_act_bits')
        return gx
    y = _c(y, 'conv output')
    assert tuple(y.shape) == g.out_shape
    check(_lib.lib().ganlab_conv_dgrad_act_f32(_p(gy), _p(y), _p(_packed(w, PACK_DGRAD, scale)), _p(gx), g.ref(), slope,
                                               _st()), 'conv_dgrad_act')
    return gx


def k_conv_fwd_mask(x, w, y, g, scale, slope):
    x, w = _c(x, 'conv input'), _c(w, 'conv weight')
    assert tuple(x.shape) == g.in_shape
    _note('fwd', g)
    out = _new(g.out_shape, x)
    if _is_bits(y):
        check(_lib.lib().ganlab_conv_fwd_mask_bits_f32(_p(x), _p(_packed(w, PACK_FWD, scale)), y.data_ptr(), _p(out), g.ref(),
                                                       slope, _st()), 'conv_fwd_mask_bits')
        return out
    y = _c(y, 'conv output')
    assert tuple(y.shape) == g.out_shape
    check(_lib.lib().ganlab_conv_fwd_mask_f32(_p(x), _p(_packed(w, PACK_FWD, scale)), _p(y), _p(out), g.ref(), slope,
                                              _st()), 'conv_fwd_mask')
    return out


def k_conv_wgrad_act(gy, y, x, g, scale, slope, bias_scale, want_gb):
    gy, x = _c(gy, 'conv grad_out'), _c(x, 'conv input')
    assert tuple(gy.shape) == g.out_shape and tuple(x.shape) == g.in_shape
    _note('wgrad', g)
    L = _lib.lib()
    gw = _take('gw', (g.Cout, g.Cin, g.ks, g.ks), x)
    gb = _take('gb', (g.Cout,), x) if want_gb else None
    ws = torch.empty((max(L.ganlab_conv_wgrad_workspace(g.ref()), 4) + 3) // 4, dtype=torch.float32, device=x.device)
    if _is_bits(y):
        check(L.ganlab_conv_wgrad_act_bits_f32(_p(gy), y.data_ptr(), _p(x), _p(gw), _p(gb), g.ref(), scale, bias_scale, slope,
                                               _p(ws), ws.numel() * 4, _st()), 'conv_wgrad_act_bits')
        return gw, gb
    y = _c(y, 'conv output')
    assert tuple(y.shape) == g.out_shape
    check(L.ganlab_conv_wgrad_act_f32(_p(gy), _p(y), _p(x), _p(gw), _p(gb), g.ref(), scale, bias_scale, slope, _p(ws),
                                      ws.numel() * 4, _st()), 'conv_wgrad_act')
    return gw, gb


def k_conv_fwd_bits(x, w, bias, g, scale, bias_scale, act, slope):
    x, w = _c(x, 'conv input'), _c(w, 'conv weight')
    assert tuple(x.shape) == g.in_shape
    _note('fwd', g)
    y = _new(g.out_shape, x)
    bits = torch.empty((y.numel() // 32,), dtype=torch.int32, device=x.device)
    check(_lib.lib().ganlab_conv_fwd_bits_f32(_p(x), _p(_packed(w, PACK_FWD, scale)), _p(_c(bias, 'bias')) if bias is not None
                                              else None, _p(y), bits.data_ptr(), g.ref(), bias_scale, act, slope, _st()),
          'conv_fwd_bits')
    return y, bits


def k_conv_fwd_blur_bits(x, w, bias, g, scale, bias_scale, slope):
    if g.ks != 3 or g.up or g.pool or g.bf is not None or get_compute_dtype() != 'f32' or not mask_bits_ok_plane():
        return None
    if os.environ.get('GANLAB_ROLL_BLUR') == '0':
        return None
    x, w = _c(x, 'conv input'), _c(w, 'conv weight')
    L = _lib.lib()
    y = _new(g.out_shape, x)
    if not L.ganlab_conv_fwd_blur_supported(g.ref(), _p(x), _p(y)):
        return None
    assert tuple(x.shape) == g.in_shape
    _note('fwd', g)
    bits = torch.empty((y.numel() // 32,), dtype=torch.int32, device=x.device)
    check(L.ganlab_conv_fwd_blur_bits_f32(_p(x), _p(_packed(w, PACK_FWD, scale)), _p(_c(bias, 'bias')) if bias is not None
                                          else None, _p(y), bits.data_ptr(), g.ref(), bias_scale, slope, _st()),
          'conv_fwd_blur_bits')
    return y, bits


def conv_s2_blur_ok(g):
    import os
    if get_compute_dtype() != 'f32' or g.bf is not None or not g.s2 or os.environ.get('GANLAB_S2_ROLL_BLUR') == '0':
        return False
    key = ('s2blur', g.N, g.Cin, g.Hin, g.Win, g.Cout, g.up, g.pool)
    hit = _AFF_OK.get(key)
    if hit is None:
        hit = bool(_lib.lib().ganlab_conv_s2_blur_supported(g.ref()))
        _AFF_OK[key] = hit
    return hit


def k_conv_s2_fwd_blur_tail(a, s_, t_, w, bias, noise, noise_w, g, scale, bias_scale, act, slope, eps):
    a, w = _c(a, 'conv input'), _c(w, 'conv weight')
    assert g.up and tuple(a.shape) == g.in_shape
    _note('fwd', g)
    L = _lib.lib()
    y = _new(g.out_shape, a)
    mean, rstd = _new((g.N, g.Cout), a), _new((g.N, g.Cout), a)
    ws = torch.empty((L.ganlab_conv_s2_blur_workspace(g.ref()) + 7) // 8, dtype=torch.float64, device=a.device)
    wp = _packed(w, PACK_FWD, scale, s2_up=1)
    noise = _c(noise) if noise is not None else None
    if noise is not None:
        assert noise.numel() == g.N * g.Ho * g.Wo, (tuple(noise.shape), g.out_shape)
    check(L.ganlab_conv_s2_fwd_blur_tail_f32(_p(a), _p(wp), _p(s_), _p(t_), _p(bias), _p(noise), _p(noise_w), _p(y), _p(mean),
                                             _p(rstd), g.ref(), bias_scale, act, slope, eps, ctypes.c_void_p(ws.data_ptr()),
                                             ws.numel() * 8, _st()), 'conv_s2_fwd_blur_tail')
    return y, mean, rstd


def k_conv_s2_dgrad_blur_act(gy, w, bits, g, scale, slope, bias_scale, want_gb):
    gy, w = _c(gy, 'conv grad_out'), _c(w, 'conv weight')
    assert g.pool and tuple(gy.shape) == g.out_shape and bits.numel() * 32 == g.N * g.Cin * g.Hin * g.Win
    _note('dgrad', g)
    L = _lib.lib()
    gz = _new(g.in_shape, gy)
    gb = _new((g.Cin,), gy) if want_gb else None
    ws = torch.empty((L.ganlab_conv_s2_blur_workspace(g.ref()) + 7) // 8, dtype=torch.float64, device=gy.device) \
        if want_gb else None
    wp = _packed(w, PACK_DGRAD, scale, s2_up=0)
    check(L.ganlab_conv_s2_dgrad_blur_act_bits_f32(_p(gy), _p(wp), bits.data_ptr(), _p(gz), _p(gb), g.ref(), slope, bias_scale,
                                                   ctypes.c_void_p(ws.data_ptr()) if ws is not None else None,
                                                   ws.numel() * 8 if ws is not None else 0, _st()),
          'conv_s2_dgrad_blur_act_bits')
    return gz, gb


def k_conv_wgrad(gy, x, g, scale):
    gy, x = _c(gy, 'conv grad_out'), _c(x, 'conv input')
    assert tuple(gy.shape) == g.out_shape and tuple(x.shape) == g.in_shape
    _note('wgrad', g)
    L = _lib.lib()
    gw = _take('gw', (g.Cout, g.Cin, g.ks, g.ks), x)
    if x3_wgrad_ok(g):
        return _wgrad_x3(gy, x, None, None, gw, g, scale)
    if g.bf is not None:
        if g.bf_fused is not None:
            nbytes = L.ganlab_conv_wgrad_bf16_workspace(ctypes.byref(g.bf_fused))
            if nbytes > 0:
                ws = torch.empty((nbytes + 3) // 4, dtype=torch.float32, device=x.device)
                check(L.ganlab_conv_wgrad_bf16(_p(gy), _p(x), _p(gw), ctypes.byref(g.bf_fused), scale, _p(ws),
# ... 1840 lines not shown
                                                           ctx.bias_scale, _p(ws), ws.numel() * 4 if ws is not None else 0,
                                                           _st()), 'instnorm_bwd_act_blur')
        else:
            check(L.ganlab_instnorm_style_bwd_act_f32(_p(gout), _p(y), _p(mean), _p(rstd), _p(style), _p(s1), _p(s2),
                                                      _p(noise) if want_nw else None, _p(gz), _p(gb), _p(gnw), n, c,
                                                      hw, ctx.act, ctx.slope, ctx.bias_scale, _p(ws),
                                                      ws.numel() * 4 if ws is not None else 0, _st()),
                  'instnorm_bwd_act')
            if blur and ctx.want_x_grad:
                gz = k_blur(gz)
    gstyle = None
    if style is not None and ctx.want_style_grad:
        gstyle = torch.stack((s2, s1), dim=1).reshape(ctx.style_shape)
    if _sunk('gb'):
        gb = None
    if _sunk('gnw'):
        gnw = None
    return gz, (gb.view(ctx.bias_shape) if gb is not None else None), \
        (gnw.view(ctx.nw_shape) if gnw is not None else None), gstyle


class _LayerTailDeferred(Function):

    @staticmethod
    def forward(ctx, x, bias, noise, noise_w, style, bias_scale, act, slope, blur, eps, link=None):
        kern = k_blur_bias_act_stats if blur else k_bias_act_stats
        noise = _c(noise) if noise is not None else None
        ctx.link = link
        y, mean, rstd = kern(x, bias, noise, noise_w, bias_scale, act, slope, eps)
        n, c, _ = _nchw(y)
        style_c = _c(style) if style is not None else None
        s_, t_ = _affine_from_stats(mean, rstd, style_c, n, c)
        ctx.save_for_backward(y, mean, rstd, style_c, noise)
        ctx.bias_scale, ctx.act, ctx.slope, ctx.blur = bias_scale, act, slope, blur
        ctx.bias_shape = bias.shape if bias is not None else None
        ctx.nw_shape = noise_w.shape if noise_w is not None else None
        ctx.bias_ref, ctx.nw_ref = bias, noise_w
        ctx.style_shape = style.shape if style is not None else None
        ctx.want_x_grad, ctx.want_bias_grad = ctx.needs_input_grad[0], ctx.needs_input_grad[1]
        ctx.want_nw_grad, ctx.want_style_grad = ctx.needs_input_grad[3], ctx.needs_input_grad[4]
        ctx.mark_non_differentiable(s_, t_, mean, rstd)
        return y, s_, t_, mean, rstd

    @staticmethod
    @once_differentiable
    def backward(ctx, g_b, *_):
        gz, gb, gnw, gstyle = _layer_tail_backward(ctx, ctx.saved_tensors, g_b, blur=ctx.blur)
        gx = gz if ctx.want_x_grad else None
        return gx, gb, None, gnw, gstyle, None, None, None, None, None, None


class _Materialize(Function):

    @staticmethod
    def forward(ctx, a, mean, rstd, style):
        n, c, hw = _nchw(a)
        out = torch.empty_like(a)
        check(_lib.lib().ganlab_instnorm_style_fwd_f32(_p(a), _p(mean), _p(rstd), _p(style), _p(out), n, c, hw, _st()),
              'instnorm_style_fwd')
        return out

    @staticmethod
    @once_differentiable
    def backward(ctx, g):
        return g, None, None, None


def materialize(x):
    if isinstance(x, Deferred):
        x.read()
        return _Materialize.apply(x.a, x.mean, x.rstd, x.style)
    return x


_AFF_OK = {}


def mod_conv_shape_ok(shape, weight, padding=1):
    if get_compute_dtype() != 'f32' or padding != 1:
        return False
    key = ('mod', tuple(int(v) for v in shape), tuple(weight.shape))
    hit = _AFF_OK.get(key)
    if hit is None:
        n, cin, h, w = key[1]
        hit = False
        if tuple(weight.shape[1:]) == (cin, 3, 3):
            g = ConvGeom(n, cin, h, w, int(weight.shape[0]), 3, 1, 0, 0)
            hit = bool(_lib.lib().ganlab_mod_conv_supported(ctypes.byref(g)))
        _AFF_OK[key] = hit
    return hit


def conv_tail_shape_ok(shape, weight, padding=1):
    if get_compute_dtype() != 'f32' or padding != 1:
        return False
    key = ('tail', tuple(int(v) for v in shape), tuple(weight.shape))
    hit = _AFF_OK.get(key)
    if hit is None:
        n, cin, h, w = key[1]
        hit = False
        if tuple(weight.shape[1:]) == (cin, 3, 3) and conv_aff_ok(shape, weight, False, padding):
            g = ConvGeom(n, cin, h, w, int(weight.shape[0]), 3, 1, 0, 0)
            hit = _lib.lib().ganlab_conv_fwd_aff_tail_chunks(ctypes.byref(g)) > 0
        _AFF_OK[key] = hit
    return hit


def mod_conv_ok(d, weight, padding=1):
    return isinstance(d, Deferred) and (mod_conv_shape_ok(d.a.shape, weight, padding) or
                                        conv_tail_shape_ok(d.a.shape, weight, padding))


def conv_aff_ok(shape, weight, up=False, padding=1):
    if get_compute_dtype() != 'f32' or padding != 1:
        return False
    key = ('up' if up else 'plain', tuple(int(v) for v in shape), tuple(weight.shape))
    hit = _AFF_OK.get(key)
    if hit is None:
        n, cin, h, w = key[1]
        hit = False
        if tuple(weight.shape[1:]) == (cin, 3, 3):
            g = ConvGeom(n, cin, h, w, int(weight.shape[0]), 3, 1, 1 if up else 0, 0)
            L = _lib.lib()
            hit = (L.ganlab_conv_s2_aff_supported(ctypes.byref(g)) if up else L.ganlab_conv_aff_supported(ctypes.byref(g))) == 3
        _AFF_OK[key] = hit
    return hit


def deferrable(x):
    import os
    if os.environ.get('GANLAB_DEFER') == '0':
        return False
    n, c, h, w = x.shape
    return get_compute_dtype() == 'f32' and h * w >= STATS_MIN_PLANE and w % 4 == 0 and h % 2 == 0


def k_conv_fwd_aff(a, s_, t_, w, g, scale):
    a, w = _c(a, 'conv input'), _c(w, 'conv weight')
    assert tuple(a.shape) == g.in_shape and tuple(s_.shape) == (g.N, g.Cin) and tuple(t_.shape) == (g.N, g.Cin)
    _note('fwd', g)
    y = _new(g.out_shape, a)
    L = _lib.lib()
    if g.up and x3_s2_ok(g):
        check(L.ganlab_conv_s2_fwd_aff_x3(_p(a), _packed_x3_s2(w, 1, scale).data_ptr(), _p(s_), _p(t_), None, _p(y), g.ref(), 1.0,
                                          ACT_NONE, 0.2, _st()), 'conv_s2_fwd_aff_x3')
    elif g.up:
        assert g.s2
        wp = _packed(w, PACK_FWD, scale, s2_up=1)
        check(L.ganlab_conv_s2_fwd_aff_f32(_p(a), _p(wp), _p(s_), _p(t_), None, _p(y), g.ref(), 1.0, ACT_NONE, 0.2, _st()),
              'conv_s2_fwd_aff')
    elif x3_ok(g):
        check(L.ganlab_conv_fwd_aff_x3(_p(a), _packed_x3(w, PACK_FWD, scale).data_ptr(), _p(s_), _p(t_), None, _p(y), g.ref(), 1.0,
                                       ACT_NONE, 0.2, _st()), 'conv_fwd_aff_x3')
    else:
        wp = _packed(w, PACK_FWD, scale)
        check(L.ganlab_conv_fwd_aff_f32(_p(a), _p(wp), _p(s_), _p(t_), None, _p(y), g.ref(), 1.0, ACT_NONE, 0.2, _st()),
              'conv_fwd_aff')
    return y


def k_conv_wgrad_aff(gy, a, s_, t_, g, scale):
    gy, a = _c(gy, 'conv grad_out'), _c(a, 'conv input')
    assert tuple(gy.shape) == g.out_shape and tuple(a.shape) == g.in_shape
    _note('wgrad', g)
    L = _lib.lib()
    gw = _take('gw', (g.Cout, g.Cin, 3, 3), a)
    if not g.up and x3_wgrad_ok(g):
        return _wgrad_x3(gy, a, _c(s_), _c(t_), gw, g, scale)
    if g.up and x3_s2_wgrad_ok(g):
        return _wgrad_x3_s2(gy, a, _c(s_), _c(t_), gw, g, scale)
    if g.up:
        ws = torch.empty((max(L.ganlab_conv_s2_wgrad_workspace(g.ref()), 4) + 3) // 4, dtype=torch.float32, device=a.device)
        check(L.ganlab_conv_s2_wgrad_aff_f32(_p(gy), _p(a), _p(s_), _p(t_), _p(gw), g.ref(), scale, _p(ws), ws.numel() * 4,
                                             _st()), 'conv_s2_wgrad_aff')
    else:
        ws = torch.empty((max(L.ganlab_conv_wgrad_workspace(g.ref()), 4) + 3) // 4, dtype=torch.float32, device=a.device)
        check(L.ganlab_conv_wgrad_aff_f32(_p(gy), _p(a), _p(s_), _p(t_), _p(gw), g.ref(), scale, _p(ws), ws.numel() * 4,
                                          _st()), 'conv_wgrad_aff')
    return gw


class _ConvAff(Function):

    @staticmethod
    def forward(ctx, a, s_, t_, w, g, scale):
        ctx.save_for_backward(a, s_, t_, w)
        ctx.g, ctx.scale = g, scale
        return k_conv_fwd_aff(a, s_, t_, w, g, scale)

    @staticmethod
    @once_differentiable
    def backward(ctx, gy):
        a, s_, t_, w = ctx.saved_tensors
        ga = k_conv_dgrad(gy, w, ctx.g, ctx.scale) if ctx.needs_input_grad[0] else None
        gw = None
        if ctx.needs_input_grad[3] and _want_param_grads():
            _sink('gw', w)
            gw = k_conv_wgrad_aff(gy, a, s_, t_, ctx.g, ctx.scale)
            if _sunk('gw'):
                gw = None
        return ga, None, None, gw, None, None


def conv_aff(d, weight, scale, up=False):
    n, cin, h, w = d.read().a.shape
    g = Geom(n, cin, h, w, weight.shape[0], 3, 1, 1 if up else 0, 0)
    return _ConvAff.apply(d.a, d.s, d.t, weight, g, float(scale))


class _ConvModTail(Function):

    @staticmethod
    def forward(ctx, a_in, s_in, t_in, w, bias, noise, noise_w, style, scale, bias_scale, act, slope, eps, link=None):
        a_in, w = _c(a_in), _c(w)
        n, cin, h, wd = a_in.shape
        cout = w.shape[0]
        L = _lib.lib()
        ctx.link = link
        g = Geom(n, cin, h, wd, cout, 3, 1, 0)
        _note('fwd', g)
        noise = _c(noise) if noise is not None else None
        y = _new((n, cout, h, wd), a_in)
        mean, rstd = _new((n, cout), a_in), _new((n, cout), a_in)
        thin = mod_conv_shape_ok(a_in.shape, w)
        if not thin and x3_ok(g):
            chunks = L.ganlab_conv_fwd_aff_tail_x3_chunks(g.ref())
            ws = torch.empty((n * cout * chunks * 2,), dtype=torch.float64, device=a_in.device)
            check(L.ganlab_conv_fwd_aff_tail_x3(_p(a_in), _packed_x3(w, PACK_FWD, scale).data_ptr(), _p(s_in), _p(t_in), _p(bias),
                                                _p(noise), _p(noise_w), _p(y), _p(mean), _p(rstd), g.ref(), bias_scale, act, slope,
                                                eps, _p(ws), ws.numel() * 8, _st()), 'conv_fwd_aff_tail_x3')
            wp = None
        else:
            wp = _packed(w, PACK_FWD, scale)
        if wp is None:
            pass
        elif thin:
            chunks = L.ganlab_mod_conv_stat_chunks(g.ref())
            ws = torch.empty((n * cout * chunks * 2,), dtype=torch.float64, device=a_in.device)
            check(L.ganlab_mod_conv_fwd_f32(_p(a_in), _p(wp), _p(s_in), _p(t_in), _p(bias), _p(noise), _p(noise_w), _p(y),
                                            _p(mean), _p(rstd), g.ref(), bias_scale, act, slope, eps, _p(ws), ws.numel() * 8,
                                            _st()), 'mod_conv_fwd')
        else:
            chunks = L.ganlab_conv_fwd_aff_tail_chunks(g.ref())
            ws = torch.empty((n * cout * chunks * 2,), dtype=torch.float64, device=a_in.device)
            check(L.ganlab_conv_fwd_aff_tail_f32(_p(a_in), _p(wp), _p(s_in), _p(t_in), _p(bias), _p(noise), _p(noise_w), _p(y),
                                                 _p(mean), _p(rstd), g.ref(), bias_scale, act, slope, eps, _p(ws),
                                                 ws.numel() * 8, _st()), 'conv_fwd_aff_tail')
        style_c = _c(style) if style is not None else None
        s_, t_ = _affine_from_stats(mean, rstd, style_c, n, cout)
        ctx.save_for_backward(a_in, s_in, t_in, w, y, mean, rstd, style_c, noise)
        ctx.g, ctx.scale = g, scale
        ctx.bias_scale, ctx.act, ctx.slope, ctx.blur = bias_scale, act, slope, False
        ctx.bias_shape = bias.shape if bias is not None else None
        ctx.nw_shape = noise_w.shape if noise_w is not None else None
        ctx.bias_ref, ctx.nw_ref = bias, noise_w
        ctx.style_shape = style.shape if style is not None else None
        ctx.want_x_grad = ctx.needs_input_grad[0] or ctx.needs_input_grad[3]
        ctx.want_bias_grad, ctx.want_nw_grad = ctx.needs_input_grad[4], ctx.needs_input_grad[6]
        ctx.want_style_grad = ctx.needs_input_grad[7]
        ctx.mark_non_differentiable(s_, t_, mean, rstd)
        return y, s_, t_, mean, rstd

    @staticmethod
    @once_differentiable
    def backward(ctx, g_b, *_):
        a_in, s_in, t_in, w = ctx.saved_tensors[:4]
        gz, gb, gnw, gstyle = _layer_tail_backward(ctx, ctx.saved_tensors[4:], g_b)
        g = ctx.g
        ga = gw = None
        if ctx.needs_input_grad[0]:
            ga = k_conv_dgrad(gz, w, g, ctx.scale)
        if ctx.needs_input_grad[3] and _want_param_grads():
            _sink('gw', w)
            gw = k_conv_wgrad_aff(gz, a_in, s_in, t_in, g, ctx.scale)
            if _sunk('gw'):
                gw = None
        return ga, None, None, gw, gb, None, gnw, gstyle, None, None, None, None, None, None


class _UpConvBlurTail(Function):

    @staticmethod
    def forward(ctx, a_in, s_in, t_in, w, bias, noise, noise_w, style, g, scale, bias_scale, act, slope, eps):
        noise = _c(noise) if noise is not None else None
        y, mean, rstd = k_conv_s2_fwd_blur_tail(a_in, s_in, t_in, w, bias, noise, noise_w, g, scale, bias_scale, act, slope,
                                                eps)
        style_c = _c(style) if style is not None else None
        s_, t_ = _affine_from_stats(mean, rstd, style_c, g.N, g.Cout)
        ctx.save_for_backward(a_in, s_in, t_in, w, y, mean, rstd, style_c, noise)
        ctx.g, ctx.scale = g, scale
        ctx.bias_scale, ctx.act, ctx.slope = bias_scale, act, slope
        ctx.bias_shape = bias.shape if bias is not None else None
        ctx.nw_shape = noise_w.shape if noise_w is not None else None
        ctx.style_shape = style.shape if style is not None else None
        ctx.bias_ref, ctx.nw_ref = bias, noise_w
        ctx.want_x_grad = ctx.needs_input_grad[0] or ctx.needs_input_grad[3]
        ctx.want_bias_grad, ctx.want_nw_grad = ctx.needs_input_grad[4], ctx.needs_input_grad[6]
        ctx.want_style_grad = ctx.needs_input_grad[7]
        ctx.mark_non_differentiable(s_, t_, mean, rstd)
        return y, s_, t_, mean, rstd

    @staticmethod
    @once_differentiable
    def backward(ctx, g_b, *_):
        a_in, s_in, t_in, w = ctx.saved_tensors[:4]
        gz, gb, gnw, gstyle = _layer_tail_backward(ctx, ctx.saved_tensors[4:], g_b, blur=True)
        g = ctx.g
        ga = gw = None
        if ctx.needs_input_grad[0]:
            ga = k_conv_dgrad(gz, w, g, ctx.scale)
        if ctx.needs_input_grad[3] and _want_param_grads():
            _sink('gw', w)
            gw = k_conv_wgrad_aff(gz, a_in, s_in, t_in, g, ctx.scale) if s_in is not None else \
                k_conv_wgrad(gz, a_in, g, ctx.scale)
            if _sunk('gw'):
                gw = None
        return ga, None, None, gw, gb, None, gnw, gstyle, None, None, None, None, None, None


def upconv_blur_tail_ok(shape, weight, deferred, padding=1):
    if padding != 1 or tuple(weight.shape[2:]) != (3, 3) or int(weight.shape[1]) != int(shape[1]):
        return False
    n, cin, h, w = (int(v) for v in shape)
    try:
        g = Geom(n, cin, h, w, int(weight.shape[0]), 3, 1, 1, 0)
    except ValueError:
        return False
    if not conv_s2_blur_ok(g) or not _lib.lib().ganlab_blur_fused_supported(2 * h, 2 * w):
        return False
    return conv_aff_ok(shape, weight, True, padding) if deferred else True


def upconv_blur_tail(x, weight, scale, bias=None, noise=None, noise_w=None, style=None, bias_scale=1.0, act=None, slope=0.2,
                     eps=1e-8):
    a_in, s_in, t_in = (x.a, x.s, x.t) if isinstance(x, Deferred) else (x, None, None)
    if isinstance(x, Deferred):
        x.read()
    n, cin, h, w = a_in.shape
    g = Geom(n, cin, h, w, weight.shape[0], 3, 1, 1, 0)
    a = ACT_LRELU if act == 'lrelu' else ACT_NONE
    y, s_, t_, mean, rstd = _UpConvBlurTail.apply(a_in, s_in, t_in, weight, bias, noise, noise_w, style, g, float(scale),
                                                  float(bias_scale), a, float(slope), float(eps))
    return Deferred(y, s_, t_, mean, rstd, style)


class _ToRGBMod(Function):

    @staticmethod
    def forward(ctx, a, s_, t_, w, bias, scale, bias_scale, link=None):
        a, w = _c(a), _c(w)
        n, cin, h, wd = a.shape
        cout = w.shape[0]
        L = _lib.lib()
        ctx.link = link
        weff, beff = _new((n, cin, 4), a), _new((n, 4), a)
        check(L.ganlab_mod_torgb_prep_f32(_p(w), _p(bias), _p(s_), _p(t_), _p(weff), _p(beff), n, cin, cout, scale,
                                          bias_scale, _st()), 'mod_torgb_prep')
        y = _new((n, cout, h, wd), a)
        check(L.ganlab_mod_torgb_fwd_f32(_p(a), _p(weff), _p(beff), _p(y), n, cin, cout, h * wd, _st()), 'mod_torgb_fwd')
        ctx.save_for_backward(a, s_, t_, w)
        ctx.scale, ctx.bias_scale = scale, bias_scale
        ctx.bias_shape = bias.shape if bias is not None else None
        ctx.bias_ref = bias
        return y

    @staticmethod
    @once_differentiable
    def backward(ctx, gy):
        a, s_, t_, w = ctx.saved_tensors
        gy = _c(gy)
        n, cin, h, wd = a.shape
        cout = w.shape[0]
        L = _lib.lib()
        g = Geom(n, cin, h, wd, cout, 1, 0, 0)
        ga = None
        if ctx.link is not None:
            ctx.link.grgb = ctx.link.wp = None
        if ctx.needs_input_grad[0]:
            link = ctx.link
            if _rgb_link_ok(link, n, cin, cout, h * wd):
                link.grgb, link.wp, link.crgb = gy, _packed(w, PACK_DGRAD, ctx.scale), cout
                ga = torch.zeros((1,), dtype=a.dtype, device=a.device).expand(a.shape)
            else:
# ... 1421 lines not shown
```

### include/ganlab_hip.h

```cpp
#ifndef GANLAB_HIP_H
#define GANLAB_HIP_H

#include <stddef.h>
#include <stdint.h>

#ifdef __cplusplus
extern "C" {
#endif

#define GANLAB_OK 0
#define GANLAB_EINVAL (-1)
#define GANLAB_EWORKSPACE (-2)
#define GANLAB_ELAUNCH (-3)
#define GANLAB_EUNSUPPORTED (-4)

#define GANLAB_ACT_NONE 0
#define GANLAB_ACT_LRELU 1

#define GANLAB_PACK_FWD 0
#define GANLAB_PACK_DGRAD 1

int ganlab_abi_version(void);

int ganlab_last_launch(char* name, int cap, unsigned* grid);
unsigned long long ganlab_launch_count(void);
int ganlab_launch_history(int back, char* name, int cap, unsigned* grid);

typedef struct {
  int N, Cin, Hin, Win;
  int Cout, ks, pad;
  int up;
  int pool;
} ganlab_conv_geom;

int ganlab_conv_geom_size(void);

int ganlab_conv_out_hw(const ganlab_conv_geom* g, int* Hout, int* Wout);

long long ganlab_conv_pack_f32(const float* w, float* out, int Cout, int Cin, int ks, int mode,
                               float scale, void* stream);

int ganlab_conv_fwd_f32(const float* x, const float* wp, const float* bias, float* y,
                        const ganlab_conv_geom* g, float bias_scale, int act, float slope,
                        void* stream);

int ganlab_conv_dgrad_f32(const float* gy, const float* wp, float* gx_virtual,
                          const ganlab_conv_geom* g, void* stream);

int ganlab_conv_splitk_plan(const ganlab_conv_geom* g, int dgrad);
int ganlab_conv_fwd_splitk_f32(const float* x, const float* wp, const float* bias, float* y, const ganlab_conv_geom* g,
                               float bias_scale, int act, float slope, void* workspace, size_t workspace_bytes,
                               void* stream);
int ganlab_conv_dgrad_splitk_f32(const float* gy, const float* wp, float* gx, const ganlab_conv_geom* g, void* workspace,
                                 size_t workspace_bytes, void* stream);

int ganlab_conv_dgrad_mask_supported(const ganlab_conv_geom* g);
int ganlab_conv_dgrad_mask_f32(const float* gy, const float* wp, const float* x, float* gx, const ganlab_conv_geom* g,
                               float slope, void* stream);

int ganlab_conv_act_bwd_fused_supported(const ganlab_conv_geom* g);
int ganlab_conv_dgrad_act_f32(const float* gy, const float* y, const float* wp, float* gx, const ganlab_conv_geom* g,
                              float slope, void* stream);
int ganlab_conv_fwd_mask_f32(const float* x, const float* wp, const float* y, float* out, const ganlab_conv_geom* g,
                             float slope, void* stream);
int ganlab_conv_wgrad_act_f32(const float* gy, const float* y, const float* x, float* gw, float* gb,
                              const ganlab_conv_geom* g, float scale, float bias_scale, float slope, void* workspace,
                              size_t workspace_bytes, void* stream);

size_t ganlab_conv_wgrad_workspace(const ganlab_conv_geom* g);
int ganlab_conv_wgrad_f32(const float* gy, const float* x, float* gw, const ganlab_conv_geom* g,
                          float scale, void* workspace, size_t workspace_bytes, void* stream);

int ganlab_conv_s2_supported(const ganlab_conv_geom* g);
long long ganlab_conv_s2_pack_f32(const float* w, float* out, int Cout, int Cin, int up, int transpose,
                                  float scale, void* stream);
int ganlab_conv_s2_fwd_f32(const float* x, const float* wp, const float* bias, float* y,
                           const ganlab_conv_geom* g, float bias_scale, int act, float slope, void* stream);
int ganlab_conv_s2_dgrad_f32(const float* gy, const float* wp, float* gx, const ganlab_conv_geom* g,
                             void* stream);
size_t ganlab_conv_s2_wgrad_workspace(const ganlab_conv_geom* g);
int ganlab_conv_s2_wgrad_f32(const float* gy, const float* x, float* gw, const ganlab_conv_geom* g,
                             float scale, void* workspace, size_t workspace_bytes, void* stream);

int ganlab_conv_bf16_supported(const ganlab_conv_geom* g);
long long ganlab_conv_pack_bf16(const float* w, void* out, int Cout, int Cin, int mode, float scale, void* stream);
int ganlab_conv_fwd_bf16(const float* x, const void* wp, const float* bias, float* y, const ganlab_conv_geom* g,
                         float bias_scale, int act, float slope, void* stream);
int ganlab_conv_dgrad_bf16(const float* gy, const void* wp, float* gx, const ganlab_conv_geom* g, void* stream);
int ganlab_conv_bf16_splitk_plan(const ganlab_conv_geom* g, int dgrad);
int ganlab_conv_fwd_bf16_splitk(const float* x, const void* wp, const float* bias, float* y, const ganlab_conv_geom* g,
                                float bias_scale, int act, float slope, void* workspace, size_t workspace_bytes,
                                void* stream);
int ganlab_conv_dgrad_bf16_splitk(const float* gy, const void* wp, float* gx, const ganlab_conv_geom* g, void* workspace,
                                  size_t workspace_bytes, void* stream);
size_t ganlab_conv_wgrad_bf16_workspace(const ganlab_conv_geom* g);
int ganlab_conv_wgrad_bf16(const float* gy, const float* x, float* gw, const ganlab_conv_geom* g, float scale,
                           void* workspace, size_t workspace_bytes, void* stream);

int ganlab_conv_x3_supported(const ganlab_conv_geom* g, int dgrad);
long long ganlab_conv_x3_pack(const float* w, void* out, int Cout, int Cin, int mode, float scale, void* stream);
int ganlab_conv_fwd_x3(const float* x, const void* wp, const float* bias, float* y, const ganlab_conv_geom* g,
                       float bias_scale, int act, float slope, void* stream);
int ganlab_conv_dgrad_x3(const float* gy, const void* wp, float* gx, const ganlab_conv_geom* g, void* stream);
int ganlab_conv_dgrad_mask_x3(const float* gy, const void* wp, const float* x, float* gx, const ganlab_conv_geom* g,
                              float slope, void* stream);
int ganlab_conv_fwd_aff_x3(const float* x, const void* wp, const float* aff_s, const float* aff_t, const float* bias,
                           float* y, const ganlab_conv_geom* g, float bias_scale, int act, float slope, void* stream);
int ganlab_conv_fwd_aff_tail_x3_chunks(const ganlab_conv_geom* g);
int ganlab_conv_s2_x3_supported(const ganlab_conv_geom* g, int dgrad);
long long ganlab_conv_s2_x3_pack(const float* w, void* out, int Cout, int Cin, int up, float scale, void* stream);
int ganlab_conv_s2_fwd_x3(const float* x, const void* wp, const float* bias, float* y, const ganlab_conv_geom* g,
                          float bias_scale, int act, float slope, void* stream);
int ganlab_conv_s2_fwd_aff_x3(const float* x, const void* wp, const float* aff_s, const float* aff_t, const float* bias,
                              float* y, const ganlab_conv_geom* g, float bias_scale, int act, float slope, void* stream);
int ganlab_conv_s2_dgrad_x3(const float* gy, const void* wp, float* gx, const ganlab_conv_geom* g, void* stream);
int ganlab_conv_s2_down_x3_supported(const ganlab_conv_geom* g, int dgrad);
long long ganlab_conv_s2_down_x3_pack(const float* w, void* out, int Cout, int Cin, int up, float scale, void* stream);
int ganlab_conv_s2_down_fwd_x3(const float* x, const void* wp, const float* bias, float* y, const ganlab_conv_geom* g,
                               float bias_scale, int act, float slope, void* stream);
int ganlab_conv_s2_down_dgrad_x3(const float* gy, const void* wp, float* gx, const ganlab_conv_geom* g, void* stream);
int ganlab_conv_wgrad_x3_supported(const ganlab_conv_geom* g);
size_t ganlab_conv_wgrad_x3_workspace(const ganlab_conv_geom* g);
int ganlab_conv_wgrad_x3(const float* gy, const float* x, const float* aff_s, const float* aff_t, float* gw,
                         const ganlab_conv_geom* g, float scale, void* workspace, size_t workspace_bytes, void* stream);
int ganlab_conv_s2_wgrad_x3_supported(const ganlab_conv_geom* g);
size_t ganlab_conv_s2_wgrad_x3_workspace(const ganlab_conv_geom* g);
int ganlab_conv_s2_wgrad_x3(const float* gy, const float* x, const float* aff_s, const float* aff_t, float* gw,
                            const ganlab_conv_geom* g, float scale, void* workspace, size_t workspace_bytes, void* stream);
int ganlab_conv_fwd_aff_tail_x3(const float* x, const void* wp, const float* aff_s, const float* aff_t, const float* bias,
                                const float* noise, const float* noise_w, float* y, float* mean, float* rstd,
                                const ganlab_conv_geom* g, float bias_scale, int act, float slope, float eps, void* workspace,
                                size_t workspace_bytes, void* stream);

int ganlab_blur3x3_f32(const float* x, float* y, long long planes, int H, int W, void* stream);
int ganlab_up2_f32(const float* x, float* y, long long planes, int H, int W, float scale, void* stream);
int ganlab_pool2_f32(const float* x, float* y, long long planes, int Hout, int Wout, float scale,
                     void* stream);
int ganlab_resample2d_f32(const float* x, float* y, const int* iy, const float* wy, const int* ix, const float* wx,
                          long long planes, int Hi, int Wi, int Ho, int Wo, int Ty, int Tx, void* stream);

int ganlab_bias_act_f32(const float* x, const float* bias, const float* noise, const float* noise_w,
                        float* y, int N, int C, long long HW, float bias_scale, int act, float slope,
                        void* stream);
int ganlab_act_bwd_f32(const float* gy, const float* y, float* gz, long long n, float slope, void* stream);
int ganlab_act_bwd_bias_f32(const float* gy, const float* y, float* gz, float* gb, int N, int C, long long HW,
                            float slope, float scale, void* workspace, size_t workspace_bytes, void* stream);
int ganlab_blur_fused_supported(int H, int W);
size_t ganlab_blur_fused_workspace(int N, int C, int H, int W);
int ganlab_blur_bias_act_f32(const float* x, const float* bias, const float* noise, const float* noise_w, float* y,
                             int N, int C, int H, int W, float bias_scale, int act, float slope, void* stream);
int ganlab_blur_act_bwd_f32(const float* g, const float* y, float* out, float* gb, int N, int C, int H, int W,
                            float slope, float bias_scale, void* workspace, size_t workspace_bytes, void* stream);
int ganlab_act_bwd_blur_f32(const float* g, const float* y, const float* noise, float* out, float* gb, float* gnw,
                            int N, int C, int H, int W, float slope, float bias_scale, void* workspace,
                            size_t workspace_bytes, void* stream);
size_t ganlab_act_stats_workspace(int N, int C, long long HW);
int ganlab_bias_act_stats_f32(const float* x, const float* bias, const float* noise, const float* noise_w, float* y,
                              float* mean, float* rstd, int N, int C, long long HW, float bias_scale, int act,
                              float slope, float eps, void* workspace, size_t workspace_bytes, void* stream);
int ganlab_blur_bias_act_stats_f32(const float* x, const float* bias, const float* noise, const float* noise_w,
                                   float* y, float* mean, float* rstd, int N, int C, int H, int W, float bias_scale,
                                   int act, float slope, float eps, void* workspace, size_t workspace_bytes,
                                   void* stream);
size_t ganlab_instnorm_bwd_act_workspace(int N, int C, long long HW);
int ganlab_instnorm_style_bwd_act_f32(const float* gy, const float* x, const float* mean, const float* rstd,
                                      const float* style, const float* s1, const float* s2, const float* noise,
                                      float* gz, float* gb, float* gnw, int N, int C, long long HW, int act,
                                      float slope, float bias_scale, void* workspace, size_t workspace_bytes,
                                      void* stream);
int ganlab_instnorm_style_bwd_act_blur_f32(const float* gy, const float* x, const float* mean, const float* rstd,
                                           const float* style, const float* s1, const float* s2, const float* noise,
                                           float* out, float* gb, float* gnw, int N, int C, int H, int W, int act,
                                           float slope, float bias_scale, void* workspace, size_t workspace_bytes,
                                           void* stream);
int ganlab_instnorm_bwd_rgb_supported(int N, int C, int crgb, long long HW);
size_t ganlab_instnorm_bwd_reduce_rgb_workspace(int N, int C, long long HW);
int ganlab_instnorm_style_bwd_reduce_rgb_f32(const float* grgb, const float* wp, int crgb, const float* x,
                                             const float* mean, const float* rstd, float* s1, float* s2, int N, int C,
                                             long long HW, void* workspace, size_t workspace_bytes, void* stream);
int ganlab_instnorm_style_bwd_act_rgb_f32(const float* grgb, const float* wp, int crgb, const float* x, const float* mean,
                                          const float* rstd, const float* style, const float* s1, const float* s2,
                                          const float* noise, float* gz, float* gb, float* gnw, int N, int C, long long HW,
                                          int act, float slope, float bias_scale, void* workspace, size_t workspace_bytes,
                                          void* stream);
int ganlab_channel_sum_f32(const float* a, const float* b_n1hw, float* out, int N, int C, long long HW,
                           float scale, void* workspace, size_t workspace_bytes, void* stream);
size_t ganlab_channel_sum_workspace(int N, int C, long long HW);

int ganlab_instnorm_stats_f32(const float* x, float* mean, float* rstd, long long planes, long long HW,
                              float eps, void* stream);
size_t ganlab_row_stats_workspace(long long rows, long long M);
int ganlab_row_stats_f32(const float* x, float* mean, float* rstd, long long rows, long long M, float eps,
                         void* workspace, size_t workspace_bytes, void* stream);
int ganlab_instnorm_style_fwd_f32(const float* x, const float* mean, const float* rstd,
                                  const float* style, float* y, int N, int C, long long HW, void* stream);
int ganlab_instnorm_style_bwd_reduce_f32(const float* gy, const float* x, const float* mean,
                                         const float* rstd, float* s1, float* s2, long long planes,
                                         long long HW, void* stream);
int ganlab_instnorm_style_bwd_apply_f32(const float* gy, const float* x, const float* mean,
                                        const float* rstd, const float* style, const float* s1,
                                        const float* s2, float* gx, int N, int C, long long HW,
                                        void* stream);
int ganlab_pixelnorm_fwd_f32(const float* x, float* y, int N, int C, long long HW, float eps, void* stream);
int ganlab_pixelnorm_bwd_f32(const float* gy, const float* x, float* gx, int N, int C, long long HW,
                             float eps, void* stream);

int ganlab_chan_affine_f32(const float* x, const float* scale, const float* shift, float* y, int N, int C,
                           long long HW, void* stream);
int ganlab_mul_f32(const float* a, const float* b, float* out, long long n, void* stream);
int ganlab_ln_affine_fwd_f32(const float* x, const float* mean, const float* rstd, const float* w, const float* b,
                             float* y, int N, long long M, int act, float slope, void* stream);
int ganlab_colscale_f32(const float* a, const float* w, float* out, int N, long long M, void* stream);
int ganlab_coldot_f32(const float* a, const float* x, const float* mean, const float* rstd, float* o1, float* o2,
                      int N, long long M, void* stream);
size_t ganlab_ln_rowsums_workspace(int N, long long M);
int ganlab_ln_rowsums_f32(const float* a, const float* wa, const float* x, const float* mean, const float* rstd,
                          const float* b2, const float* w2, float* out, int N, long long M, void* workspace,
                          size_t workspace_bytes, const float* yact, float* gz, float slope, void* stream);
int ganlab_ln_project_f32(const float* a, const float* wa, const float* x, const float* mean, const float* rstd,
                          const float* sums, const float* wo, float* out, int N, long long M, void* stream);
int ganlab_ln_bwd_cols_f32(const float* a, const float* w, const float* x, const float* mean, const float* rstd,
                           const float* sums, float* gx, float* gw, float* gb, int N, long long M, void* stream);
int ganlab_ln_bwdbwd_apply_f32(const float* x, const float* mean, const float* rstd, const float* pu, const float* gx,
                               const float* sums, const float* usums, float* out, int N, long long M, void* stream);
int ganlab_bn_stats_f32(const float* x, float* out, int N, int C, long long HW, void* workspace, size_t workspace_bytes,
                        void* stream);
int ganlab_bn_apply_f32(const float* x, const float* mean, const float* scale, const float* shift, float* y, int N,
                        int C, long long HW, int act, float slope, void* stream);
int ganlab_bn_finalize_f32(const float* mom, const float* weight, float* running_mean, float* running_var,
                           long long* batches, float* out, int C, float eps, float momentum, float unbias,
                           void* stream);
int ganlab_bn_bwd_sums_f32(const float* gy, const float* x, const float* mean, const float* rstd, float* out, int N,
                           int C, long long HW, void* workspace, size_t workspace_bytes, const float* yact, float* gz,
                           float slope, void* stream);
int ganlab_bn_bwd_apply_f32(const float* gy, const float* x, const float* mean, const float* rstd, const float* sums,
                            const float* pre, float* gx, int N, int C, long long HW, void* stream);
int ganlab_tanh_fwd_f32(const float* x, float* y, long long n, void* stream);
int ganlab_tanh_bwd_f32(const float* gy, const float* y, float* gx, long long n, void* stream);

int ganlab_mbstd_fwd_f32(const float* x, float* stat, int G, int gs, long long F, float eps, void* stream);
int ganlab_mbstd_bwd_f32(const float* x, const float* gstat, float* gx, int G, int gs, long long F,
                         float eps, void* stream);
int ganlab_mbstd_bwdbwd_f32(const float* x, const float* gstat, const float* ggx, float* g_gstat,
                            float* g_x, int G, int gs, long long F, float eps, void* stream);

int ganlab_axpby_f32(const float* x, const float* y, float* out, long long n, float a, float b, void* stream);
int ganlab_scale_dev_f32(const float* x, const float* gout, float* out, long long n, float a, void* stream);
int ganlab_lerp_rows_f32(const float* a, const float* b, const float* t, float* out, long long N, long long M,
                         void* stream);
int ganlab_sum_f32(const float* x, float* out, long long n, float scale, int squared, void* workspace,
                   size_t workspace_bytes, void* stream);
size_t ganlab_sum_workspace(long long n);
int ganlab_bce_logits_fwd_f32(const float* x, float* out, int n, float target, void* stream);
int ganlab_bce_logits_bwd_f32(const float* x, const float* gout, float* gx, int n, float target, void* stream);
int ganlab_hinge_fwd_f32(const float* x, float* out, int n, float a, float b, void* stream);
int ganlab_hinge_bwd_f32(const float* x, const float* gout, float* gx, int n, float a, float b, void* stream);
int ganlab_chnorm_penalty_fwd_f32(const float* g, float* out, int N, int C, long long HW, float gamma,
                                  float scale, void* workspace, size_t workspace_bytes, void* stream);
int ganlab_chnorm_penalty_bwd_f32(const float* g, const float* gout, float* gg, int N, int C, long long HW,
                                  float gamma, float scale, void* stream);

// ... 295 lines not shown
```

Measured before the change: 168.9 images/sec.

## Add thin 32-channel split-bf16 MFMA conv kernel for high-resolution 3x3 layers

Adds a specialised persistent 3x3 convolution kernel for Cin=Cout=32 layers that uses three-way bf16 splitting with MFMA. It keeps all nine weight taps resident in LDS and pipelines input tiles across a rotating triple buffer. It is routed for forward, dgrad, masked dgrad and affine-forward paths when there are enough tiles, replacing the generic fp32 path for the 1024^2 layers. The fused norm-tail variant stays behind an env flag. Precision relies on the bf16x3 split emulating fp32.

```diff
diff --git a/gan_lab_amd/_lib.py b/gan_lab_amd/_lib.py
--- a/gan_lab_amd/_lib.py
+++ b/gan_lab_amd/_lib.py
@@ -97,6 +97,15 @@
     'ganlab_conv_dgrad_mask_x3': (_c_int, [_c_p, _c_p, _c_p, _c_p, _GP, _c_f, _c_p]),
     'ganlab_conv_fwd_aff_x3': (_c_int, [_c_p, _c_p, _c_p, _c_p, _c_p, _c_p, _GP, _c_f, _c_int, _c_f, _c_p]),
     'ganlab_conv_fwd_aff_tail_x3_chunks': (_c_int, [_GP]),
+    'ganlab_conv_x3t_supported': (_c_int, [_GP, _c_int]),
+    'ganlab_conv_x3t_pack': (_c_ll, [_c_p, _c_p, _c_int, _c_int, _c_int, _c_f, _c_p]),
+    'ganlab_conv_fwd_x3t': (_c_int, [_c_p, _c_p, _c_p, _c_p, _GP, _c_f, _c_int, _c_f, _c_int, _c_p]),
+    'ganlab_conv_dgrad_x3t': (_c_int, [_c_p, _c_p, _c_p, _GP, _c_int, _c_p]),
+    'ganlab_conv_dgrad_mask_x3t': (_c_int, [_c_p, _c_p, _c_p, _c_p, _GP, _c_f, _c_int, _c_p]),
+    'ganlab_conv_fwd_aff_x3t': (_c_int, [_c_p, _c_p, _c_p, _c_p, _c_p, _c_p, _GP, _c_f, _c_int, _c_f, _c_int, _c_p]),
+    'ganlab_conv_fwd_aff_tail_x3t_chunks': (_c_int, [_GP]),
+    'ganlab_conv_fwd_aff_tail_x3t': (_c_int, [_c_p, _c_p, _c_p, _c_p, _c_p, _c_p, _c_p, _c_p, _c_p, _c_p, _GP, _c_f, _c_int, _c_f,
+                                              _c_f, _c_p, _c_sz, _c_int, _c_p]),
     'ganlab_conv_s2_x3_supported': (_c_int, [_GP, _c_int]),
     'ganlab_conv_s2_x3_pack': (_c_ll, [_c_p, _c_p, _c_int, _c_int, _c_int, _c_f, _c_p]),
     'ganlab_conv_s2_fwd_x3': (_c_int, [_c_p, _c_p, _c_p, _c_p, _GP, _c_f, _c_int, _c_f, _c_p]),
diff --git a/gan_lab_amd/csrc/common.h b/gan_lab_amd/csrc/common.h
--- a/gan_lab_amd/csrc/common.h
+++ b/gan_lab_amd/csrc/common.h
@@ -126,6 +126,24 @@
   }
 }
 
+__device__ __forceinline__ void gl_x3t_pack_position(const float* __restrict__ w9, bool flip, float scale, __bf16* __restrict__ out,
+                                                     int ci, int co) {
+  const int half = (ci >> 4) & 1, g = (ci >> 3) & 1, j = ci & 7;
+#pragma unroll
+  for (int t = 0; t < 9; ++t) {
+    const int s = t < 8 ? (half ? 5 : 0) + (t >> 1) : 4;
+    const int hi = t < 8 ? (t & 1) : half;
+    const int kg = hi * 2 + g;
+    float v = w9[flip ? 8 - t : t] * scale;
+    asm volatile("" : "+v"(v));
+    const gl_bf16x3 p = gl_split3(v);
+    __bf16* base = out + (long long)s * (3 * 4 * 32) * 8;
+    base[((0 * 4 + kg) * 32 + co) * 8 + j] = p.h;
+    base[((1 * 4 + kg) * 32 + co) * 8 + j] = p.m;
+    base[((2 * 4 + kg) * 32 + co) * 8 + j] = p.l;
+  }
+}
+
 __device__ __forceinline__ void gl_x3_up_pack_position(const float* __restrict__ w9, int up, float scale, __bf16* __restrict__ out,
                                                        int CI, int CO, int ci, int co) {
   const int nsteps = CI / 8;
diff --git a/gan_lab_amd/csrc/conv_x3.hip b/gan_lab_amd/csrc/conv_x3.hip
--- a/gan_lab_amd/csrc/conv_x3.hip
+++ b/gan_lab_amd/csrc/conv_x3.hip
@@ -16,10 +16,6 @@
 constexpr int X3_WSTAGE = 2 * X3_WSTEP;
 constexpr int X3_LDS = 3 * X3_HALF + 2 * X3_WSTAGE;
 
-__host__ __device__ constexpr int x3_tap_lo(int s) { return s < 4 ? 2 * s : s == 4 ? 8 : 2 * (s - 5); }
-__host__ __device__ constexpr int x3_tap_hi(int s) { return s < 4 ? 2 * s + 1 : s == 4 ? 8 : 2 * (s - 5) + 1; }
-__host__ __device__ constexpr int x3_half_lo(int s) { return s <= 4 ? 0 : 1; }
-__host__ __device__ constexpr int x3_half_hi(int s) { return s < 4 ? 0 : 1; }
 
 __global__ void x3_pack_kernel(const float* __restrict__ w, __bf16* __restrict__ out, int Cout, int Cin, int mode, float scale) {
   const bool dg = mode == GANLAB_PACK_DGRAD;
@@ -55,8 +51,6 @@
 constexpr int X3_PLAIN = 0, X3_MASK = 1, X3_AFF = 2, X3_AFF_TAIL = 3;
 
 #define X3_ACC8(a) "+v"(a[0][0]), "+v"(a[0][1]), "+v"(a[1][0]), "+v"(a[1][1]), "+v"(a[2][0]), "+v"(a[2][1]), "+v"(a[3][0]), "+v"(a[3][1])
-
-__host__ __device__ constexpr int x3_toff(int tap) { return (tap / 3) * 18 + tap % 3; }
 
 struct X3Tile { int n, oy0, ox0, co_t; };
 
diff --git a/gan_lab_amd/csrc/conv_x3_thin.hip b/gan_lab_amd/csrc/conv_x3_thin.hip
--- /dev/null
+++ b/gan_lab_amd/csrc/conv_x3_thin.hip
@@ -0,0 +1,357 @@
+#include "x3_common.h"
+
+namespace {
+
+constexpr int XT_PL = 336;
+constexpr int XT_HALF = 6 * XT_PL;
+constexpr int XT_WSTEP = 3 * 4 * 32;
+constexpr int XT_WOFF = 3 * XT_HALF;
+constexpr int XT_DUMMY = 3 * XT_HALF + 9 * XT_WSTEP;
+constexpr int XT_LDS = XT_DUMMY + 256;
+constexpr int XT_WAVES = 8;
+
+__global__ void x3t_pack_kernel(const float* __restrict__ w, __bf16* __restrict__ out, int mode, float scale) {
+  const bool dg = mode == GANLAB_PACK_DGRAD;
+  const int e = blockIdx.x * blockDim.x + threadIdx.x;
+  if (e >= 32 * 32) return;
+  const int co = e & 31, ci = e >> 5;
+  const float* w9 = dg ? w + (ci * 32 + co) * 9 : w + (co * 32 + ci) * 9;
+  gl_x3t_pack_position(w9, dg, scale, out, ci, co);
+}
+
+struct XtArgs {
+  const float* x;
+  const u32x4* wp;
+  const float* bias;
+  float* y;
+  int N, H, W;
+  int tiles_x, tiles_y, ntiles;
+  float bias_scale, slope;
+  int act;
+  const float* mask;
+  float mslope;
+  const float* aff_s;
+  const float* aff_t;
+  const float* noise;
+  const float* noise_w;
+  double* spart;
+};
+
+constexpr int XT_PLAIN = 0, XT_MASK = 1, XT_AFF = 2, XT_AFF_TAIL = 3;
+
+struct XtTile { int n, oy0, ox0; };
+
+template <int FORM>
+__global__ __launch_bounds__(512) void conv_x3_thin_kernel(XtArgs p) {
+  constexpr bool MASK = FORM == XT_MASK, AFF = FORM == XT_AFF || FORM == XT_AFF_TAIL, TAIL = FORM == XT_AFF_TAIL;
+  constexpr int CI = 32, CO = 32;
+  __shared__ __attribute__((aligned(16))) u32x4 lds[XT_LDS];
+
+  const int tid = threadIdx.x, lane = tid & 63;
+  const int wv = __builtin_amdgcn_readfirstlane(tid >> 6);
+  const int l16 = lane & 15, kg = lane >> 4;
+  const int plane = p.H * p.W;
+  const int G = gridDim.x;
+
+  auto decode = [&](int t) {
+    XtTile c;
+    c.ox0 = (t % p.tiles_x) * 16; t /= p.tiles_x;
+    c.oy0 = (t % p.tiles_y) * 16;
+    c.n = t / p.tiles_y;
+    return c;
+  };
+
+  const bool a_item = tid < 432;
+  int a_dst, a_i0, a_i1, a_ry, a_rx, a_ch;
+  {
+    const int e = a_item ? tid : 0;
+    const int cq = e & 1;
+    int t = e >> 1;
+    const int cg = t % 6; t /= 6;
+    const int r = t % 18, g = t / 18;
+    a_dst = ((g * 3) * XT_PL + r * 18 + 4 * cg - 3) * 16 + cq * 8;
+    a_i0 = cg == 0 ? 3 : 0; a_i1 = cg == 5 ? 1 : 4;
+    a_ry = r - 1; a_rx = cg * 4 - 4; a_ch = (g * 2 + cq) * 4;
+  }
+  auto a_ok = [&](const XtTile& c) {
+    return a_item && (unsigned)(c.oy0 + a_ry) < (unsigned)p.H && (unsigned)(c.ox0 + a_rx) < (unsigned)p.W;
+  };
+  f32x4 ar[2][4];
+  f32x4 a_sv[2], a_tv[2];
+  auto a_load = [&](int set, const XtTile& c, int half, bool valid) {
+    const __amdgpu_buffer_rsrc_t rs = __builtin_amdgcn_make_buffer_rsrc(
+        const_cast<float*>(p.x + (long long)c.n * CI * plane), 0, CI * plane * 4, 0x00020000);
+    const int off = valid && a_ok(c) ? ((half * 16 + a_ch) * plane + (c.oy0 + a_ry) * p.W + c.ox0 + a_rx) * 4 : (int)0x80000000;
+#pragma unroll
+    for (int j = 0; j < 4; ++j)
+      ar[set][j] = __builtin_bit_cast(f32x4, __builtin_amdgcn_raw_buffer_load_b128(rs, off + j * plane * 4, 0, 0));
+    if constexpr (AFF) {
+      const int o = c.n * CI + half * 16 + a_ch;
+      a_sv[set] = *reinterpret_cast<const f32x4*>(p.aff_s + o);
+      a_tv[set] = *reinterpret_cast<const f32x4*>(p.aff_t + o);
+    }
+  };
+  auto a_store_px = [&](int set, const XtTile& c, int slot, int i) {
+    const bool keep = a_item && i >= a_i0 && i < a_i1;
+    unsigned char* const base = reinterpret_cast<unsigned char*>(lds);
+    unsigned char* dst = base + (keep ? slot * 16 + a_dst + i * 16 : XT_DUMMY * 16 + tid * 8);
+    const int pstep = keep ? XT_PL * 16 : 0;
+    const bool ok = a_ok(c);
+    bf16x4 h, m, l;
+#pragma unroll
+    for (int j = 0; j < 4; ++j) {
+      float v = ar[set][j][i];
+      if constexpr (AFF) v = ok ? fmaf(v, a_sv[set][j], a_tv[set][j]) : 0.f;
+      x3_split_lane(v, j, h, m, l);
+    }
+    *reinterpret_cast<u32x2*>(dst) = __builtin_bit_cast(u32x2, h);
+    *reinterpret_cast<u32x2*>(dst + pstep) = __builtin_bit_cast(u32x2, m);
+    *reinterpret_cast<u32x2*>(dst + 2 * pstep) = __builtin_bit_cast(u32x2, l);
+  };
+  auto lds_barrier = [&]() { asm volatile("s_waitcnt lgkmcnt(0)\n\ts_barrier" ::: "memory"); };
+
+  f32x4 accS[2][2], accH[2][2];
+#pragma unroll
+  for (int m = 0; m < 2; ++m)
+#pragma unroll
+    for (int nn = 0; nn < 2; ++nn) { accS[m][nn] = f32x4{0.f, 0.f, 0.f, 0.f}; accH[m][nn] = f32x4{0.f, 0.f, 0.f, 0.f}; }
+
+  const int laneA = (kg & 1) * 3 * XT_PL + (2 * wv) * 18 + l16;
+  const int laneB = XT_WOFF + kg * 32 + l16;
+  const bool khi = kg >= 2;
+
+  bf16x8 aF[2][2][3], bF[2][2][3];
+  auto frags = [&](int set, int s, int h0, int h1) {
+    const int u_lo = (x3_half_lo(s) ? h1 : h0) + x3_toff(x3_tap_lo(s)), u_hi = (x3_half_hi(s) ? h1 : h0) + x3_toff(x3_tap_hi(s));
+    const int off = laneA + (khi ? u_hi : u_lo);
+#pragma unroll
+    for (int m = 0; m < 2; ++m)
+#pragma unroll
+      for (int pl = 0; pl < 3; ++pl) aF[set][m][pl] = __builtin_bit_cast(bf16x8, lds[off + pl * XT_PL + m * 18]);
+#pragma unroll
+    for (int nn = 0; nn < 2; ++nn)
+#pragma unroll
+      for (int pl = 0; pl < 3; ++pl)
+        bF[set][nn][pl] = __builtin_bit_cast(bf16x8, lds[laneB + s * XT_WSTEP + pl * 4 * 32 + nn * 16]);
+  };
+
+  float bv[2], nwv[2];
+#pragma unroll
+  for (int nn = 0; nn < 2; ++nn) {
+    const int co = nn * 16 + l16;
+    bv[nn] = p.bias != nullptr ? p.bias[co] * p.bias_scale : 0.f;
+    nwv[nn] = 0.f;
+    if constexpr (TAIL) nwv[nn] = p.noise != nullptr ? p.noise_w[co] : 0.f;
+  }
+
+  int tile = gl_xcd_remap(blockIdx.x, G);
+  if (tile >= p.ntiles) return;
+  XtTile cur = decode(tile);
+  bool nvalid = tile + G < p.ntiles;
+  XtTile nxt = decode(nvalid ? tile + G : tile);
+
+  a_load(0, cur, 0, true);
+  a_load(1, cur, 1, true);
+  for (int u = tid; u < 9 * XT_WSTEP; u += 512) lds[XT_WOFF + u] = p.wp[u];
+#pragma unroll
+  for (int i = 0; i < 4; ++i) a_store_px(0, cur, 0, i);
+#pragma unroll
+  for (int i = 0; i < 4; ++i) a_store_px(1, cur, XT_HALF, i);
+  a_load(0, nxt, 0, nvalid);
+  lds_barrier();
+  frags(0, 0, 0, XT_HALF);
+
+  int sA = 0, sB = XT_HALF, sC = 2 * XT_HALF;
+  for (;;) {
+    const bool n2valid = nvalid && tile + 2 * G < p.ntiles;
+    const XtTile nx2 = decode(n2valid ? tile + 2 * G : tile);
+    f32x4 mks[MASK ? 2 : 1][MASK ? 2 : 1];
+    float4 nzs[TAIL ? 2 : 1];
+    const long long ib = (long long)cur.n * CO * plane;
+    const int px0 = (cur.oy0 + 2 * wv) * p.W + cur.ox0 + 4 * kg;
+
+    a_load(1, nxt, 1, nvalid);
+    __builtin_amdgcn_sched_barrier(0);
+#pragma unroll
+    for (int s = 0; s < 9; ++s) {
+      const int cb = s & 1;
+      if (s == 4 || s == 8) lds_barrier();
+      if (s < 8) frags(cb ^ 1, s + 1, sA, sB);
+#pragma unroll
+      for (int m = 0; m < 2; ++m)
+#pragma unroll
+        for (int nn = 0; nn < 2; ++nn) {
+          accS[m][nn] = __builtin_amdgcn_mfma_f32_16x16x32_bf16(aF[cb][m][2], bF[cb][nn][0], accS[m][nn], 0, 0, 0);
+          accS[m][nn] = __builtin_amdgcn_mfma_f32_16x16x32_bf16(aF[cb][m][0], bF[cb][nn][2], accS[m][nn], 0, 0, 0);
+          accS[m][nn] = __builtin_amdgcn_mfma_f32_16x16x32_bf16(aF[cb][m][1], bF[cb][nn][1], accS[m][nn], 0, 0, 0);
+          accS[m][nn] = __builtin_amdgcn_mfma_f32_16x16x32_bf16(aF[cb][m][1], bF[cb][nn][0], accS[m][nn], 0, 0, 0);
+          accS[m][nn] = __builtin_amdgcn_mfma_f32_16x16x32_bf16(aF[cb][m][0], bF[cb][nn][1], accS[m][nn], 0, 0, 0);
+          accH[m][nn] = __builtin_amdgcn_mfma_f32_16x16x32_bf16(aF[cb][m][0], bF[cb][nn][0], accH[m][nn], 0, 0, 0);
+        }
+      if (s == 8) frags(0, 0, sC, sA);
+      if (s < 4) a_store_px(0, nxt, sC, s);
+      if (s >= 4 && s < 8) a_store_px(1, nxt, sA, s - 4);
+      if (s == 4) {
+#pragma unroll
+        for (int m = 0; m < 2; ++m) {
+          if constexpr (TAIL)
+            nzs[m] = p.noise != nullptr ? *reinterpret_cast<const float4*>(p.noise + (long long)cur.n * plane + px0 + m * p.W)
+                                        : float4{0.f, 0.f, 0.f, 0.f};
+          if constexpr (MASK) {
+#pragma unroll
+            for (int nn = 0; nn < 2; ++nn)
+              mks[m][nn] = *reinterpret_cast<const f32x4*>(p.mask + ib + (long long)(nn * 16 + l16) * plane + px0 + m * p.W);
+          }
+        }
+        a_load(0, nx2, 0, n2valid);
+      }
+      __builtin_amdgcn_sched_barrier(0);
+    }
+
+    {
+      float s1[2] = {0.f, 0.f}, s2[2] = {0.f, 0.f};
+#pragma unroll
+      for (int m = 0; m < 2; ++m)
+#pragma unroll
+        for (int nn = 0; nn < 2; ++nn) {
+          const int co = nn * 16 + l16;
+          const long long o = ib + (long long)co * plane + px0 + m * p.W;
+          f32x4 v = accH[m][nn] + accS[m][nn];
+#pragma unroll
+          for (int r = 0; r < 4; ++r) {
+            float f;
+            if constexpr (TAIL) f = fmaf(r == 0 ? nzs[m].x : r == 1 ? nzs[m].y : r == 2 ? nzs[m].z : nzs[m].w, nwv[nn], v[r] + bv[nn]);
+            else f = v[r] + bv[nn];
+            if (p.act == GANLAB_ACT_LRELU) f = gl_lrelu(f, p.slope);
+            if constexpr (MASK) { if (!(mks[m][nn][r] > 0.f)) f *= p.mslope; }
+            v[r] = f;
+          }
+          *reinterpret_cast<f32x4*>(p.y + o) = v;
+          if constexpr (TAIL) {
+            s1[nn] += (v[0] + v[1]) + (v[2] + v[3]);
+            s2[nn] += fmaf(v[0], v[0], v[1] * v[1]) + fmaf(v[2], v[2], v[3] * v[3]);
+          }
+          accH[m][nn] = f32x4{0.f, 0.f, 0.f, 0.f};
+          accS[m][nn] = f32x4{0.f, 0.f, 0.f, 0.f};
+        }
+      if constexpr (TAIL) {
+        const long long chunks = (long long)p.tiles_x * p.tiles_y * XT_WAVES;
+        const long long tl = ((long long)(cur.oy0 >> 4) * p.tiles_x + (cur.ox0 >> 4)) * XT_WAVES + wv;
+#pragma unroll
+        for (int nn = 0; nn < 2; ++nn) {
+          double a = (double)s1[nn], b = (double)s2[nn];
+          a += __shfl_xor(a, 16, 64); a += __shfl_xor(a, 32, 64);
+          b += __shfl_xor(b, 16, 64); b += __shfl_xor(b, 32, 64);
+          if (kg == 0) {
+            double* dst = p.spart + (((long long)cur.n * CO + nn * 16 + l16) * chunks + tl) * 2;
+            dst[0] = a; dst[1] = b;
+          }
+        }
+      }
+    }
+    if (!nvalid) break;
+    tile += G;
+    cur = nxt; nxt = nx2; nvalid = n2valid;
+    const int t = sA; sA = sC; sC = sB; sB = t;
+    __builtin_amdgcn_sched_barrier(0);
+  }
+}
+
+long long x3t_tiles(int N, int H, int W) {
+  if (N <= 0 || H <= 0 || W <= 0 || H % 16 != 0 || W % 16 != 0) return 0;
+  const long long ntiles = (long long)N * (W / 16) * (H / 16);
+  const bool fits = ntiles <= 0x3fffffffLL && 32LL * H * W * 4 <= 0x7fffffffLL && (long long)N * 32 * 4 <= 0x7fffffffLL;
+  return fits ? ntiles : 0;
+}
+
+bool x3t_ok(const ganlab_conv_geom* g) {
+  if (g == nullptr || g->ks != 3 || g->pad != 1 || g->up || g->pool) return false;
+  if (g->Cin != 32 || g->Cout != 32) return false;
+  return x3t_tiles(g->N, g->Hin, g->Win) > 0;
+}
+
+int x3t_launch(int form, XtArgs a, int max_workgroups, hipStream_t st) {
+  const long long ntiles = x3t_tiles(a.N, a.H, a.W);
+  if (ntiles <= 0 || max_workgroups < 0) return GANLAB_EINVAL;
+  a.tiles_x = a.W / 16; a.tiles_y = a.H / 16; a.ntiles = (int)ntiles;
+  long long grid = ntiles < 256 ? ntiles : 256;
+  if (max_workgroups > 0 && max_workgroups < grid) grid = max_workgroups;
+  switch (form) {
+    case XT_PLAIN: GL_LAUNCH(conv_x3_thin_kernel<XT_PLAIN>, dim3((unsigned)grid), dim3(512), 0, st, a); break;
+    case XT_MASK: GL_LAUNCH(conv_x3_thin_kernel<XT_MASK>, dim3((unsigned)grid), dim3(512), 0, st, a); break;
+    case XT_AFF: GL_LAUNCH(conv_x3_thin_kernel<XT_AFF>, dim3((unsigned)grid), dim3(512), 0, st, a); break;
+    default: GL_LAUNCH(conv_x3_thin_kernel<XT_AFF_TAIL>, dim3((unsigned)grid), dim3(512), 0, st, a); break;
+  }
+  return GL_CHECK_LAUNCH();
+}
+
+XtArgs x3t_args(const float* x, const void* wp, const float* bias, float* y, const ganlab_conv_geom* g, float bias_scale, int act,
+                float slope) {
+  XtArgs a{};
+  a.x = x; a.wp = reinterpret_cast<const u32x4*>(wp); a.bias = bias; a.y = y;
+  a.N = g->N; a.H = g->Hin; a.W = g->Win;
+  a.bias_scale = bias_scale; a.slope = slope; a.act = act;
+  return a;
+}
+
+}
+
+extern "C" {
+
+int ganlab_conv_x3t_supported(const ganlab_conv_geom* g, int dgrad) { (void)dgrad; return x3t_ok(g) ? 1 : 0; }
+
+long long ganlab_conv_x3t_pack(const float* w, void* out, int Cout, int Cin, int mode, float scale, void* stream) {
+  if (Cout != 32 || Cin != 32 || (mode != GANLAB_PACK_FWD && mode != GANLAB_PACK_DGRAD)) return GANLAB_EINVAL;
+  const long long n = 3LL * 9 * 32 * 32;
+  if (out == nullptr) return n;
+  if (w == nullptr) return GANLAB_EINVAL;
+  GL_LAUNCH(x3t_pack_kernel, dim3(4), dim3(256), 0, gl_stream(stream), w, reinterpret_cast<__bf16*>(out), mode, scale);
+  const int st = GL_CHECK_LAUNCH();
+  return st != GANLAB_OK ? st : n;
+}
+
+int ganlab_conv_fwd_x3t(const float* x, const void* wp, const float* bias, float* y, const ganlab_conv_geom* g, float bias_scale,
+                        int act, float slope, int max_workgroups, void* stream) {
+  if (!x3t_ok(g) || x == nullptr || wp == nullptr || y == nullptr) return GANLAB_EINVAL;
+  return x3t_launch(XT_PLAIN, x3t_args(x, wp, bias, y, g, bias_scale, act, slope), max_workgroups, gl_stream(stream));
+}
+
+int ganlab_conv_dgrad_x3t(const float* gy, const void* wp, float* gx, const ganlab_conv_geom* g, int max_workgroups, void* stream) {
+  if (!x3t_ok(g) || gy == nullptr || wp == nullptr || gx == nullptr) return GANLAB_EINVAL;
+  return x3t_launch(XT_PLAIN, x3t_args(gy, wp, nullptr, gx, g, 1.f, GANLAB_ACT_NONE, 0.f), max_workgroups, gl_stream(stream));
+}
+
+int ganlab_conv_dgrad_mask_x3t(const float* gy, const void* wp, const float* x, float* gx, const ganlab_conv_geom* g, float slope,
+                               int max_workgroups, void* stream) {
+  if (!x3t_ok(g) || gy == nullptr || wp == nullptr || gx == nullptr || x == nullptr) return GANLAB_EINVAL;
+  XtArgs a = x3t_args(gy, wp, nullptr, gx, g, 1.f, GANLAB_ACT_NONE, 0.f);
+  a.mask = x; a.mslope = slope;
+  return x3t_launch(XT_MASK, a, max_workgroups, gl_stream(stream));
+}
+
+int ganlab_conv_fwd_aff_x3t(const float* x, const void* wp, const float* aff_s, const float* aff_t, const float* bias, float* y,
+                            const ganlab_conv_geom* g, float bias_scale, int act, float slope, int max_workgroups, void* stream) {
+  if (!x3t_ok(g) || x == nullptr || wp == nullptr || y == nullptr || aff_s == nullptr || aff_t == nullptr) return GANLAB_EINVAL;
+  XtArgs a = x3t_args(x, wp, bias, y, g, bias_scale, act, slope);
+  a.aff_s = aff_s; a.aff_t = aff_t;
+  return x3t_launch(XT_AFF, a, max_workgroups, gl_stream(stream));
+}
+
+int ganlab_conv_fwd_aff_tail_x3t_chunks(const ganlab_conv_geom* g) { return x3t_ok(g) ? (g->Hin / 16) * (g->Win / 16) * XT_WAVES : 0; }
+int ganlab_conv_fwd_aff_tail_x3t(const float* x, const void* wp, const float* aff_s, const float* aff_t, const float* bias,
+                                 const float* noise, const float* noise_w, float* y, float* mean, float* rstd,
+                                 const ganlab_conv_geom* g, float bias_scale, int act, float slope, float eps, void* workspace,
+                                 size_t workspace_bytes, int max_workgroups, void* stream) {
+  const int chunks = ganlab_conv_fwd_aff_tail_x3t_chunks(g);
+  if (chunks <= 0) return GANLAB_EUNSUPPORTED;
+  if (!x || !wp || !y || !aff_s || !aff_t || !mean || !rstd || (noise && !noise_w)) return GANLAB_EINVAL;
+  const long long planes = (long long)g->N * g->Cout;
+  if (!workspace || workspace_bytes < (size_t)planes * chunks * 2 * sizeof(double)) return GANLAB_EWORKSPACE;
+  XtArgs a = x3t_args(x, wp, bias, y, g, bias_scale, act, slope);
+  a.aff_s = aff_s; a.aff_t = aff_t; a.noise = noise; a.noise_w = noise_w; a.spart = reinterpret_cast<double*>(workspace);
+  const int rc = x3t_launch(XT_AFF_TAIL, a, max_workgroups, gl_stream(stream));
+  if (rc != GANLAB_OK) return rc;
+  return gl_tail_stats_finish(a.spart, mean, rstd, planes, chunks, 1.0 / ((double)g->Hin * g->Win), eps, gl_stream(stream));
+}
+
+}
diff --git a/gan_lab_amd/csrc/pack.hip b/gan_lab_amd/csrc/pack.hip
--- a/gan_lab_amd/csrc/pack.hip
+++ b/gan_lab_amd/csrc/pack.hip
@@ -77,6 +77,12 @@
     const int co = ct * 128 + col;
     const float* w9 = up ? w + ((long long)ci * d.Cin + co) * 9 : w + ((long long)co * d.Cin + ci) * 9;
     gl_x3_down_pack_position(w9, up, d.scale, reinterpret_cast<__bf16*>(d.dst), CI, ci, co);
+  } else if (d.kind == GANLAB_PACKKIND_X3 && d.ks == 2) {
+    const bool dg = d.mode == GANLAB_PACK_DGRAD;
+    if (e >= 32 * 32) return;
+    const int co = (int)(e & 31), ci = (int)(e >> 5);
+    const float* w9 = dg ? w + (ci * 32 + co) * 9 : w + (co * 32 + ci) * 9;
+    gl_x3t_pack_position(w9, dg, d.scale, reinterpret_cast<__bf16*>(d.dst), ci, co);
   } else if (d.kind == GANLAB_PACKKIND_X3) {
     const bool dg = d.mode == GANLAB_PACK_DGRAD;
     const int CO = dg ? d.Cin : d.Cout, CI = dg ? d.Cout : d.Cin;
diff --git a/gan_lab_amd/csrc/x3_common.h b/gan_lab_amd/csrc/x3_common.h
--- a/gan_lab_amd/csrc/x3_common.h
+++ b/gan_lab_amd/csrc/x3_common.h
@@ -44,6 +44,12 @@
 #define X3_DRAIN(...) asm volatile("s_nop 15\n\ts_nop 15" : __VA_ARGS__)
 #define X3_SETTLE(...) asm volatile("s_nop 7\n\ts_nop 7" : __VA_ARGS__)
 
+__host__ __device__ constexpr int x3_tap_lo(int s) { return s < 4 ? 2 * s : s == 4 ? 8 : 2 * (s - 5); }
+__host__ __device__ constexpr int x3_tap_hi(int s) { return s < 4 ? 2 * s + 1 : s == 4 ? 8 : 2 * (s - 5) + 1; }
+__host__ __device__ constexpr int x3_half_lo(int s) { return s <= 4 ? 0 : 1; }
+__host__ __device__ constexpr int x3_half_hi(int s) { return s < 4 ? 0 : 1; }
+__host__ __device__ constexpr int x3_toff(int tap) { return (tap / 3) * 18 + tap % 3; }
+
 __device__ __forceinline__ void x3_split_lane(float v, int j, bf16x4& h, bf16x4& m, bf16x4& l) {
   h[j] = (__bf16)v;
   const float r1 = v - (float)h[j];
diff --git a/gan_lab_amd/ops.py b/gan_lab_amd/ops.py
--- a/gan_lab_amd/ops.py
+++ b/gan_lab_amd/ops.py
@@ -207,6 +207,8 @@
         rc = L.ganlab_conv_s2_x3_pack(_p(e.w), e.out.data_ptr(), cout, cin, up, scale, _st())
     elif kind == _KIND_X3 and ks == 5:
         rc = L.ganlab_conv_s2_down_x3_pack(_p(e.w), e.out.data_ptr(), cout, cin, up, scale, _st())
+    elif kind == _KIND_X3 and ks == 2:
+        rc = L.ganlab_conv_x3t_pack(_p(e.w), e.out.data_ptr(), cout, cin, mode, scale, _st())
     elif kind == _KIND_X3:
         rc = L.ganlab_conv_x3_pack(_p(e.w), e.out.data_ptr(), cout, cin, mode, scale, _st())
     else:
@@ -340,6 +342,19 @@
     return bool(_lib.lib().ganlab_conv_x3_supported(g.ref(), 1 if dgrad else 0))
 
 
+_X3T_MIN_TILES = 256
+_X3T_MAX_WORKGROUPS = [0]
+_X3T_TAIL = [os.environ.get('GANLAB_X3T_TAIL', '0') == '1']
+
+
+def x3t_ok(g, dgrad=False):
+    if not _X3[0] or g.bf is not None or g.s2 or g.up or g.pool or g.ks != 3 or g.pad != 1 or g.Cin != 32 or g.Cout != 32:
+        return False
+    if g.N * (g.Hin // 16) * (g.Win // 16) < _X3T_MIN_TILES:
+        return False
+    return bool(_lib.lib().ganlab_conv_x3t_supported(g.ref(), 1 if dgrad else 0))
+
+
 def x3_s2_ok(g, dgrad=False):
     if not _X3[0] or not g.s2:
         return False
@@ -406,7 +421,7 @@
     rc = pack(_p(w), out.data_ptr(), cout, cin, sel, scale, _st())
     if rc != n:
         raise _lib.GanlabLibraryError(f'{name} failed ({rc})')
-    mode, up = (sel, 0) if ks == 3 else (0, sel)
+    mode, up = (sel, 0) if ks in (2, 3) else (0, sel)
     return _pack_store(key, w, out, (_KIND_X3, cout, cin, ks, mode, up, float(scale), int(n)))
 
 
@@ -420,6 +435,10 @@
 
 def _packed_x3(w, mode, scale):
     return _packed_x3_any('conv_x3_pack', 'x3', w, mode, scale, 3)
+
+
+def _packed_x3t(w, mode, scale):
+    return _packed_x3_any('conv_x3t_pack', 'x3t', w, mode, scale, 2)
 
 
 _INPUT_GRAD_ONLY = [False]
@@ -592,6 +611,10 @@
         check(L.ganlab_conv_fwd_x3(_p(x), _packed_x3(w, PACK_FWD, scale).data_ptr(), _p(bias), _p(y), g.ref(), bias_scale, act,
                                    slope, _st()), 'conv_fwd_x3')
         return y
+    if x3t_ok(g):
+        check(L.ganlab_conv_fwd_x3t(_p(x), _packed_x3t(w, PACK_FWD, scale).data_ptr(), _p(bias), _p(y), g.ref(), bias_scale, act,
+                                    slope, _X3T_MAX_WORKGROUPS[0], _st()), 'conv_fwd_x3t')
+        return y
     wp = _packed(w, PACK_FWD, scale)
     split = 0 if g.up else L.ganlab_conv_splitk_plan(g.ref(), 0)
     if split >= 2:
@@ -646,6 +669,11 @@
         check(_lib.lib().ganlab_conv_dgrad_x3(_p(gy), _packed_x3(w, PACK_DGRAD, scale).data_ptr(), _p(gx), g.ref(), _st()),
               'conv_dgrad_x3')
         return gx
+    if x3t_ok(g, True):
+        gx = _new(g.in_shape, gy)
+        check(_lib.lib().ganlab_conv_dgrad_x3t(_p(gy), _packed_x3t(w, PACK_DGRAD, scale).data_ptr(), _p(gx), g.ref(),
+                                               _X3T_MAX_WORKGROUPS[0], _st()), 'conv_dgrad_x3t')
+        return gx
     wp = _packed(w, PACK_DGRAD, scale)
     hv, wv = (2 * g.Hin, 2 * g.Win) if g.up else (g.Hin, g.Win)
     gxv = _new((g.N, g.Cin, hv, wv), gy)
@@ -673,6 +701,10 @@
     if x3_ok(g, True):
         check(_lib.lib().ganlab_conv_dgrad_mask_x3(_p(gy), _packed_x3(w, PACK_DGRAD, scale).data_ptr(), _p(x), _p(gx), g.ref(),
                                                    slope, _st()), 'conv_dgrad_mask_x3')
+        return gx
+    if x3t_ok(g, True):
+        check(_lib.lib().ganlab_conv_dgrad_mask_x3t(_p(gy), _packed_x3t(w, PACK_DGRAD, scale).data_ptr(), _p(x), _p(gx), g.ref(),
+                                                    slope, _X3T_MAX_WORKGROUPS[0], _st()), 'conv_dgrad_mask_x3t')
         return gx
     check(_lib.lib().ganlab_conv_dgrad_mask_f32(_p(gy), _p(_packed(w, PACK_DGRAD, scale)), _p(x), _p(gx), g.ref(), slope,
                                                 _st()), 'conv_dgrad_mask')
@@ -2819,6 +2851,9 @@
     elif x3_ok(g):
         check(L.ganlab_conv_fwd_aff_x3(_p(a), _packed_x3(w, PACK_FWD, scale).data_ptr(), _p(s_), _p(t_), None, _p(y), g.ref(), 1.0,
                                        ACT_NONE, 0.2, _st()), 'conv_fwd_aff_x3')
+    elif x3t_ok(g):
+        check(L.ganlab_conv_fwd_aff_x3t(_p(a), _packed_x3t(w, PACK_FWD, scale).data_ptr(), _p(s_), _p(t_), None, _p(y), g.ref(), 1.0,
+                                        ACT_NONE, 0.2, _X3T_MAX_WORKGROUPS[0], _st()), 'conv_fwd_aff_x3t')
     else:
         wp = _packed(w, PACK_FWD, scale)
         check(L.ganlab_conv_fwd_aff_f32(_p(a), _p(wp), _p(s_), _p(t_), None, _p(y), g.ref(), 1.0, ACT_NONE, 0.2, _st()),
@@ -2896,6 +2931,14 @@
             check(L.ganlab_conv_fwd_aff_tail_x3(_p(a_in), _packed_x3(w, PACK_FWD, scale).data_ptr(), _p(s_in), _p(t_in), _p(bias),
                                                 _p(noise), _p(noise_w), _p(y), _p(mean), _p(rstd), g.ref(), bias_scale, act, slope,
                                                 eps, _p(ws), ws.numel() * 8, _st()), 'conv_fwd_aff_tail_x3')
+            wp = None
+        elif not thin and _X3T_TAIL[0] and x3t_ok(g):
+            chunks = L.ganlab_conv_fwd_aff_tail_x3t_chunks(g.ref())
+            ws = torch.empty((n * cout * chunks * 2,), dtype=torch.float64, device=a_in.device)
+            check(L.ganlab_conv_fwd_aff_tail_x3t(_p(a_in), _packed_x3t(w, PACK_FWD, scale).data_ptr(), _p(s_in), _p(t_in), _p(bias),
+                                                 _p(noise), _p(noise_w), _p(y), _p(mean), _p(rstd), g.ref(), bias_scale, act, slope,
+                                                 eps, _p(ws), ws.numel() * 8, _X3T_MAX_WORKGROUPS[0], _st()),
+                  'conv_fwd_aff_tail_x3t')
             wp = None
         else:
             wp = _packed(w, PACK_FWD, scale)
diff --git a/include/ganlab_hip.h b/include/ganlab_hip.h
--- a/include/ganlab_hip.h
+++ b/include/ganlab_hip.h
@@ -107,6 +107,22 @@
 int ganlab_conv_fwd_aff_x3(const float* x, const void* wp, const float* aff_s, const float* aff_t, const float* bias,
                            float* y, const ganlab_conv_geom* g, float bias_scale, int act, float slope, void* stream);
 int ganlab_conv_fwd_aff_tail_x3_chunks(const ganlab_conv_geom* g);
+int ganlab_conv_x3t_supported(const ganlab_conv_geom* g, int dgrad);
+long long ganlab_conv_x3t_pack(const float* w, void* out, int Cout, int Cin, int mode, float scale, void* stream);
+int ganlab_conv_fwd_x3t(const float* x, const void* wp, const float* bias, float* y, const ganlab_conv_geom* g,
+                        float bias_scale, int act, float slope, int max_workgroups, void* stream);
+int ganlab_conv_dgrad_x3t(const float* gy, const void* wp, float* gx, const ganlab_conv_geom* g, int max_workgroups,
+                          void* stream);
+int ganlab_conv_dgrad_mask_x3t(const float* gy, const void* wp, const float* x, float* gx, const ganlab_conv_geom* g,
+                               float slope, int max_workgroups, void* stream);
+int ganlab_conv_fwd_aff_x3t(const float* x, const void* wp, const float* aff_s, const float* aff_t, const float* bias,
+                            float* y, const ganlab_conv_geom* g, float bias_scale, int act, float slope, int max_workgroups,
+                            void* stream);
+int ganlab_conv_fwd_aff_tail_x3t_chunks(const ganlab_conv_geom* g);
+int ganlab_conv_fwd_aff_tail_x3t(const float* x, const void* wp, const float* aff_s, const float* aff_t, const float* bias,
+                                 const float* noise, const float* noise_w, float* y, float* mean, float* rstd,
+                                 const ganlab_conv_geom* g, float bias_scale, int act, float slope, float eps, void* workspace,
+                                 size_t workspace_bytes, int max_workgroups, void* stream);
 int ganlab_conv_s2_x3_supported(const ganlab_conv_geom* g, int dgrad);
 long long ganlab_conv_s2_x3_pack(const float* w, void* out, int Cout, int Cin, int up, float scale, void* stream);
 int ganlab_conv_s2_fwd_x3(const float* x, const void* wp, const float* bias, float* y, const ganlab_conv_geom* g,
```

After: 169.6 images/sec, median of 6. No clear change (+0.4%).
